# marcemq/crowdmod-ddpm-4D

Hardware: AMD Instinct MI355X
Metric: denoise-steps/sec (UNet fwd + sampler update) at ATC [B,4,T,H,W] (higher is better)
Workload: dtype f32; 1 GPU; config/ATC.yml sampling on the 12x36 grid, fp32 arithmetic (fp32 matrix instructions; fp32 products built from f16 two-way splits -- three v_mfma_f32_32x32x16_f16 cross terms, fp32 accumulate, same error against the reference as round 3's six-term bf16 form -- in the Winograd / quarter-resolution / last-conv layers, whose input is GroupNorm + SiLU output, and in the upsample layers, whose raw inpu; channels=4, past_len=5, future_len=3, global_batch=64, parallelism=batch-shard x1 (2 stream lanes of 32 chains per rank)

## Files before the change

crowdmod-ddpm-4d_amd/csrc/cm_conv_fin.hip:

```cpp
#include "cm_kernels.h"

#include <algorithm>
#include <cstring>
#include <vector>

namespace cm {

typedef float f32x16 __attribute__((ext_vector_type(16)));
typedef float f32x4 __attribute__((ext_vector_type(4)));
typedef __bf16 bf16x8 __attribute__((ext_vector_type(8)));
typedef _Float16 f16x8 __attribute__((ext_vector_type(8)));
typedef _Float16 f16x4 __attribute__((ext_vector_type(4)));

__device__ __forceinline__ float silu_f2(float v) { return v * __builtin_amdgcn_rcpf(1.0f + __expf(-v)); }

constexpr int FIN_ROWS = 64;
constexpr int FIN_PCOLS = 132;

template <int MODE>
__global__ __launch_bounds__(256, 2) void conv_fin_kernel(const ConvArgs a, const float *__restrict__ wfin, int ntx) {
  constexpr bool F16 = MODE == 1, H2 = MODE == 3;
  constexpr int U0 = MODE >= 2 ? 3 : 0, NTW = MODE >= 2 ? 2 : 3;
  constexpr int NTM = F16 ? 1 : 3;
  constexpr int RW = F16 ? 4 : 12;
  extern __shared__ __attribute__((aligned(16))) float lds[];
  float *A = lds;
  float *P = A + 4 * FIN_ROWS * RW;
  float *OACC = P + FIN_ROWS * FIN_PCOLS;
  const int tid = threadIdx.x, lane = tid & 63;
  const int wave = __builtin_amdgcn_readfirstlane(tid >> 6);
  const int r = lane & 31, hh = lane >> 5;
  const int BY = a.by, BX = a.bx, HX = BX + 2, HV = (BY + 2) * HX, NV = BY * BX;
  int tile = blockIdx.x;
  const int ntp = a.nty * ntx;
  const int b = tile / ntp, p = tile - b * ntp;
  const int ty = p / ntx, tx = p - ty * ntx;
  const int y0 = ty * BY, x0 = tx * BX;
  const size_t Vp = (size_t)a.Ys * a.Xs;
  const int C = a.C0;

  const int q = tid & 7;
  int soff[2];
  bool sok[2];
#pragma unroll
  for (int k = 0; k < 2; ++k) {
    const int hv = (tid >> 3) + 32 * k;
    const int hy = hv / HX, hx = hv - hy * HX;
    const int cy = y0 - 1 + hy, cx = x0 - 1 + hx;
    sok[k] = hv < HV && cy >= 0 && cy < a.Ys && cx >= 0 && cx < a.Xs;
    soff[k] = sok[k] ? cy * a.Xs + cx : 0;
  }
  f32x4 sc = {1.f, 1.f, 1.f, 1.f}, sh = {0.f, 0.f, 0.f, 0.f};
  if (a.gn) {
    const float *g = a.gn + (size_t)b * 2 * C + 4 * q;
    sc = *reinterpret_cast<const f32x4 *>(g);
    sh = *reinterpret_cast<const f32x4 *>(g + C);
  }
  const bool h16 = (a.h16 & 1) != 0;
  f32x4 ld[2];
  auto issue = [&](int z) {
    if (h16) {
      const _Float16 *sp = reinterpret_cast<const _Float16 *>(a.src0) + ((size_t)(b * a.Zs + z) * Vp) * C + 4 * q;
#pragma unroll
      for (int k = 0; k < 2; ++k) {
        const cm_f32x2_t two = *reinterpret_cast<const cm_f32x2_t *>(sp + (size_t)soff[k] * C);
        const f16x4 hv4 = __builtin_bit_cast(f16x4, two);
        ld[k] = f32x4{(float)hv4[0], (float)hv4[1], (float)hv4[2], (float)hv4[3]};
      }
    } else {
      const float *sp = a.src0 + ((size_t)(b * a.Zs + z) * Vp) * C + 4 * q;
#pragma unroll
      for (int k = 0; k < 2; ++k) ld[k] = *reinterpret_cast<const f32x4 *>(sp + (size_t)soff[k] * C);
    }
  };
  auto stage = [&]() {
#pragma unroll
    for (int k = 0; k < 2; ++k) {
      const int hv = (tid >> 3) + 32 * k;
      f32x4 w = ld[k];
      if (a.gn) {
        w = w * sc + sh;
        if (a.silu) { w[0] = silu_f2(w[0]); w[1] = silu_f2(w[1]); w[2] = silu_f2(w[2]); w[3] = silu_f2(w[3]); }
      }
      if (!sok[k]) w = f32x4{0.f, 0.f, 0.f, 0.f};
      float *dst = A + (size_t)(((q >> 1) & 1) * FIN_ROWS + hv) * RW + 2 * (q & 1) + (q >> 2) * (2 * FIN_ROWS * RW);
      if constexpr (F16) {
        const f16x4 hv4 = {(_Float16)w[0], (_Float16)w[1], (_Float16)w[2], (_Float16)w[3]};
        *reinterpret_cast<f16x4 *>(dst) = hv4;
      } else {
        cm_u32x2_t t3[3];
        if constexpr (H2) cm_split2_f16(w, t3);
        else cm_split3_bf16<NTW>(w, t3);
#pragma unroll
        for (int tm = 0; tm < NTW; ++tm) *reinterpret_cast<cm_u32x2_t *>(dst + 4 * tm) = t3[tm];
      }
    }
  };

  f32x4 bw[2][NTM];
#pragma unroll
  for (int ks = 0; ks < 2; ++ks)
#pragma unroll
    for (int tm = 0; tm < NTM; ++tm) bw[ks][tm] = reinterpret_cast<const f32x4 *>(wfin)[((size_t)(wave * 2 + ks) * NTM + tm) * 64 + lane];

  const int gu = tid & 63, dzg = tid >> 6;
  const bool gath = gu < NV && dzg < 3;
  const int guy = gu / BX, gux = gu - guy * BX;
  const int grow = guy * HX + gux;
  const int oy = y0 + guy, ox = x0 + gux;
  const bool oin = gath && oy < a.Yo && ox < a.Xo;
  f32x4 bias4 = {0.f, 0.f, 0.f, 0.f};
  if (gath && dzg >= 1) {
#pragma unroll
    for (int c = 0; c < 4; ++c) bias4[c] = c < a.Co ? a.bias[c] : 0.f;
  }
  for (int i = tid; i < 3 * 64 * 4; i += 256) OACC[i] = 0.f;

  const int Z = a.Zs;
  constexpr int TA[6] = {0, 2, 1, 0, 1, 0}, TB[6] = {2, 0, 1, 1, 0, 0};
  issue(0);
  stage();
  if (Z > 1) issue(1);
  __syncthreads();
  for (int z = 0; z < Z; ++z) {
    f32x16 acc[2];
#pragma unroll
    for (int j = 0; j < 2; ++j)
#pragma unroll
      for (int e = 0; e < 16; ++e) acc[j][e] = 0.f;
#pragma unroll
    for (int ks = 0; ks < 2; ++ks)
#pragma unroll
      for (int j = 0; j < 2; ++j) {
        const float *ap = A + (size_t)ks * (2 * FIN_ROWS * RW) + (size_t)(hh * FIN_ROWS + 32 * j + r) * RW;
        if constexpr (F16) {
          const f32x4 af = *reinterpret_cast<const f32x4 *>(ap);
          acc[j] = __builtin_amdgcn_mfma_f32_32x32x16_f16(__builtin_bit_cast(f16x8, bw[ks][0]), __builtin_bit_cast(f16x8, af), acc[j], 0, 0, 0);
        } else {
          f32x4 af[3];
#pragma unroll
          for (int tm = 0; tm < 3; ++tm) af[tm] = *reinterpret_cast<const f32x4 *>(ap + 4 * tm);
#pragma unroll
          for (int u = U0; u < 6; ++u) {
            if constexpr (H2)
              acc[j] = __builtin_amdgcn_mfma_f32_32x32x16_f16(__builtin_bit_cast(f16x8, bw[ks][TB[u]]), __builtin_bit_cast(f16x8, af[TA[u]]), acc[j], 0, 0, 0);
            else
              acc[j] = __builtin_amdgcn_mfma_f32_32x32x16_bf16(__builtin_bit_cast(bf16x8, bw[ks][TB[u]]), __builtin_bit_cast(bf16x8, af[TA[u]]), acc[j], 0, 0, 0);
          }
        }
      }
#pragma unroll
    for (int j = 0; j < 2; ++j)
#pragma unroll
      for (int g = 0; g < 4; ++g) {
        f32x4 pv = f32x4{acc[j][4 * g], acc[j][4 * g + 1], acc[j][4 * g + 2], acc[j][4 * g + 3]};
        if constexpr (H2) pv = pv * a.h2_oscale;
        *reinterpret_cast<f32x4 *>(P + (size_t)(32 * j + r) * FIN_PCOLS + 4 * (8 * wave + 2 * g + hh)) = pv;
      }
    __syncthreads();
    if (z + 1 < Z) {
      stage();
      if (z + 2 < Z) issue(z + 2);
    }
    if (gath) {
      const int zo = z + 1 - dzg;
      if (zo >= 0 && zo < a.Zo) {
        f32x4 s4 = {0.f, 0.f, 0.f, 0.f};
#pragma unroll
        for (int t9 = 0; t9 < 9; ++t9) {
          const int dy = t9 / 3, dx = t9 - 3 * dy;
          s4 += *reinterpret_cast<const f32x4 *>(P + (size_t)(grow + dy * HX + dx) * FIN_PCOLS + 4 * (dzg * 9 + t9));
        }
        float *oa = OACC + (size_t)(((zo % 3) * 64 + gu) * 4);
        f32x4 v = *reinterpret_cast<const f32x4 *>(oa) + s4;
        const bool last = dzg == 2 || (dzg == 1 && z == Z - 1);
        if (last) {
          if (oin) {
            float *o = a.out + ((size_t)((b * a.Zo + zo) * a.Yo + oy) * a.Xo + ox) * a.out_cs;
#pragma unroll
            for (int c = 0; c < 4; ++c)
              if (c < a.Co) o[c] = v[c] + bias4[c];
          }
          v = f32x4{0.f, 0.f, 0.f, 0.f};
        }
        *reinterpret_cast<f32x4 *>(oa) = v;
      }
    }
    __syncthreads();
  }
}

bool conv_fin_pick(int Y, int X, int *by, int *bx) {
  double best = 0;
  for (int y = 1; y <= Y; ++y)
    for (int x = 1; x <= X; ++x) {
      if (Y % y || X % x) continue;
      const int hv = (y + 2) * (x + 2);
      if (hv > FIN_ROWS || y * x > 64) continue;
      const double score = (double)(y * x) / FIN_ROWS;
      if (score > best) { best = score; *by = y; *bx = x; }
    }
  return best > 0;
}

bool conv_fin_ok(const ConvArgs &a) {
  return a.ntaps == 27 && a.td == 3 && a.stride == 1 && !a.par && !a.ups && a.C0 == 32 && a.C1 == 0 && a.Co >= 1 && a.Co <= 4 && !a.temb &&
         !a.resid && !a.stat_part && !a.pm && a.ks <= 1 && a.out_cs >= a.Co && a.Zs == a.Zo && a.Ys == a.Yo && a.Xs == a.Xo && a.by > 0 &&
         a.bx > 0 && a.Yo % a.by == 0 && a.Xo % a.bx == 0 && (a.by + 2) * (a.bx + 2) <= FIN_ROWS && a.by * a.bx <= 64 && !(a.h16 & ~1);
}

size_t conv_fin_lds(bool f16) {
  return ((size_t)2 * 2 * FIN_ROWS * (f16 ? 4 : 12) + (size_t)FIN_ROWS * FIN_PCOLS + 3 * 64 * 4) * sizeof(float);
}

hipError_t launch_conv_fin(const ConvArgs &a_in, const float *wfin, int mode, hipStream_t st) {
  ConvArgs a = a_in;
  a.dbg = conv_dbg_flags();
  if (!conv_fin_ok(a) || mode < 0 || mode > 3) return hipErrorInvalidValue;
  const int nty = a.Yo / a.by, ntx = a.Xo / a.bx;
  a.nty = nty;
  const dim3 grid((unsigned)(a.B * nty * ntx));
  const size_t lds = conv_fin_lds(mode == 1);
  static bool attr_set[64][4] = {{false}};
  int dev = 0;
  (void)hipGetDevice(&dev);
  const void *fn = mode == 1 ? reinterpret_cast<const void *>(conv_fin_kernel<1>)
                 : mode == 2 ? reinterpret_cast<const void *>(conv_fin_kernel<2>)
                 : mode == 3 ? reinterpret_cast<const void *>(conv_fin_kernel<3>) : reinterpret_cast<const void *>(conv_fin_kernel<0>);
  if (!attr_set[dev & 63][mode]) {
    hipError_t e = hipFuncSetAttribute(fn, hipFuncAttributeMaxDynamicSharedMemorySize, 160 * 1024);
    if (e != hipSuccess) return e;
    attr_set[dev & 63][mode] = true;
  }
  if (mode == 1) hipLaunchKernelGGL(conv_fin_kernel<1>, grid, dim3(256), lds, st, a, wfin, ntx);
  else if (mode == 2) hipLaunchKernelGGL(conv_fin_kernel<2>, grid, dim3(256), lds, st, a, wfin, ntx);
  else if (mode == 3) hipLaunchKernelGGL(conv_fin_kernel<3>, grid, dim3(256), lds, st, a, wfin, ntx);
  else hipLaunchKernelGGL(conv_fin_kernel<0>, grid, dim3(256), lds, st, a, wfin, ntx);
  return hipGetLastError();
}

__global__ __launch_bounds__(256) void fin_pack_kernel(const float *__restrict__ w, unsigned short *__restrict__ out, int Co, int f16, float wscale) {
  const int o = blockIdx.x * 256 + threadIdx.x;
  if (o >= 4 * 2 * 64 * 8) return;
  const int j = o & 7, lane = (o >> 3) & 63, ks = (o >> 9) & 1, nb = o >> 10;
  const int n = 32 * nb + (lane & 31), t = n >> 2, co = n & 3, ci = 16 * ks + 8 * (lane >> 5) + j;
  float v = 0.f;
  if (t < 27 && co < Co) {
    const int dz = t / 9, dy = (t / 3) % 3, dx = t % 3;
    v = w[((size_t)co * 32 + ci) * 27 + (dy * 3 + dx) * 3 + dz];
  }
  const int ntm = f16 == 1 ? 1 : 3;
  const size_t base = (((size_t)(nb * 2 + ks) * ntm) * 64 + lane) * 8 + j;
  if (f16 == 2) {
    const float vs = v * wscale;
    const _Float16 h = (_Float16)vs;
    const _Float16 md = (_Float16)(vs - (float)h);
    out[base] = __builtin_bit_cast(unsigned short, h);
    out[base + (size_t)64 * 8] = __builtin_bit_cast(unsigned short, md);
    out[base + (size_t)2 * 64 * 8] = 0;
  } else if (f16) {
    const _Float16 h = (_Float16)v;
    out[base] = __builtin_bit_cast(unsigned short, h);
  } else {
    float rem = v;
#pragma unroll
    for (int tm = 0; tm < 3; ++tm) {
      const __bf16 h = (__bf16)rem;
      out[base + (size_t)tm * 64 * 8] = __builtin_bit_cast(unsigned short, h);
      rem -= (float)h;
    }
  }
}

hipError_t launch_fin_pack(const float *w_ref, float *wfin, int Co, int mode, hipStream_t st, float wscale) {
  hipLaunchKernelGGL(fin_pack_kernel, dim3(16), dim3(256), 0, st, w_ref, reinterpret_cast<unsigned short *>(wfin), Co, mode, wscale);
  return hipGetLastError();
}

}
```

crowdmod-ddpm-4d_amd/csrc/cm_conv_io.hip:

```cpp
#include "cm_kernels.h"

namespace cm {

typedef float f32x16 __attribute__((ext_vector_type(16)));
typedef float f32x4 __attribute__((ext_vector_type(4)));
typedef float f32x2 __attribute__((ext_vector_type(2)));

template <int CIN>
__global__ __launch_bounds__(256) void conv_first_kernel(const ConvArgs a, const float *__restrict__ wpk, int nblk) {
  constexpr int NS = 27 * CIN / 2;
  constexpr int HC = CIN / 2;
  extern __shared__ __attribute__((aligned(16))) float lds[];
  const int tid = threadIdx.x, lane = tid & 63;
  const int wave = __builtin_amdgcn_readfirstlane(tid >> 6);
  const int r = lane & 31, hh = lane >> 5;
  int tile = blockIdx.x;
  if (!(gridDim.x & 7) && !(a.dbg & 4096)) tile = (tile & 7) * (int)(gridDim.x >> 3) + (tile >> 3);
  const int ty = tile % a.nty; tile /= a.nty;
  const int tz = tile % a.ntz;
  const int b = tile / a.ntz;
  const int nt = blockIdx.y;
  const int X = a.Xo, bz = a.bz, by = a.by;
  const int z0 = tz * bz, y0 = ty * by;
  const int HY = by + 2, HX = X + 2;
  const int HV = (bz + 2) * HY * HX;
  const int nbox = bz * by * X;

  int *outoff = reinterpret_cast<int *>(lds);
  float *P0 = lds + 32 * nblk;

  float wreg[NS];
  {
    const float *wp = wpk + (size_t)nt * NS * 64 + lane;
#pragma unroll
    for (int s = 0; s < NS; ++s) wreg[s] = wp[s * 64];
  }
  constexpr int SU = 4;
  for (int hv0 = tid; hv0 < HV; hv0 += 256 * SU) {
    f32x4 v0[SU], v1[CIN == 8 ? SU : 1];
    bool okv[SU];
#pragma unroll
    for (int u = 0; u < SU; ++u) {
      const int hv = min(hv0 + 256 * u, HV - 1);
      const int hz = hv / (HY * HX), rem = hv - hz * (HY * HX), hy = rem / HX, hx = rem - hy * HX;
      const int cz = z0 + hz - 1, cy = y0 + hy - 1, cx = hx - 1;
      const bool ok = cz >= 0 && cz < a.Zs && cy >= 0 && cy < a.Ys && cx >= 0 && cx < a.Xs;
      const float *sp = a.src0 + ((size_t)((b * a.Zs + (ok ? cz : 0)) * a.Ys + (ok ? cy : 0)) * a.Xs + (ok ? cx : 0)) * a.C0;
      v0[u] = *reinterpret_cast<const f32x4 *>(sp);
      if constexpr (CIN == 8) v1[u] = *reinterpret_cast<const f32x4 *>(sp + 4);
      okv[u] = ok;
    }
#pragma unroll
    for (int u = 0; u < SU; ++u) {
      const int hv = hv0 + 256 * u;
      if (hv >= HV) continue;
      const f32x4 z4 = {0.f, 0.f, 0.f, 0.f};
      const f32x4 w0 = okv[u] ? v0[u] : z4;
      if constexpr (CIN == 4) {
        *reinterpret_cast<f32x2 *>(P0 + hv * 2) = f32x2{w0[0], w0[1]};
        *reinterpret_cast<f32x2 *>(P0 + (HV + hv) * 2) = f32x2{w0[2], w0[3]};
      } else {
        const f32x4 w1 = okv[u] ? v1[u] : z4;
        *reinterpret_cast<f32x4 *>(P0 + hv * 4) = w0;
        *reinterpret_cast<f32x4 *>(P0 + (HV + hv) * 4) = w1;
      }
    }
  }
  for (int m = tid; m < 32 * nblk; m += 256) {
    int off = -1;
    if (m < nbox) {
      const int z = m / (by * X), rem = m - z * (by * X), y = rem / X, x = rem - y * X;
      const int oz = z0 + z, oy = y0 + y;
      if (oz < a.Zo && oy < a.Yo && b < a.B) off = ((b * a.Zo + oz) * a.Yo + oy) * a.Xo + x;
    }
    outoff[m] = off;
  }
  __syncthreads();

  const float *Ph = P0 + (size_t)hh * HV * HC;
  const int n = nt * 32 + r;
  const bool nok = n < a.Co;
  const float bias = a.bias[nok ? n : 0];
  for (int blk = wave; blk < nblk; blk += 4) {
    const int m = min(blk * 32 + r, nbox - 1);
    const int z = m / (by * X), rem = m - z * (by * X), y = rem / X, x = rem - y * X;
    const float *ap = Ph + (size_t)((z * HY + y) * HX + x) * HC;
    f32x16 acc;
#pragma unroll
    for (int i = 0; i < 16; ++i) acc[i] = 0.f;
#pragma unroll
    for (int t = 0; t < 27; ++t) {
      const int dz = t / 9, dy = (t / 3) % 3, dx = t % 3;
      const int toff = ((dz * HY + dy) * HX + dx) * HC;
      if constexpr (CIN == 4) {
        const f32x2 v = *reinterpret_cast<const f32x2 *>(ap + toff);
        acc = __builtin_amdgcn_mfma_f32_32x32x2f32(v[0], wreg[2 * t], acc, 0, 0, 0);
        acc = __builtin_amdgcn_mfma_f32_32x32x2f32(v[1], wreg[2 * t + 1], acc, 0, 0, 0);
      } else {
        const f32x4 v = *reinterpret_cast<const f32x4 *>(ap + toff);
#pragma unroll
        for (int jj = 0; jj < 4; ++jj) acc = __builtin_amdgcn_mfma_f32_32x32x2f32(v[jj], wreg[4 * t + jj], acc, 0, 0, 0);
      }
    }
    int offs[16];
    float rs[16];
#pragma unroll
    for (int reg = 0; reg < 16; ++reg) offs[reg] = outoff[blk * 32 + (reg & 3) + 8 * (reg >> 2) + 4 * hh];
#pragma unroll
    for (int reg = 0; reg < 16; ++reg) rs[reg] = acc[reg] + bias;
    if (a.h16 & 4) {
      _Float16 *oh = reinterpret_cast<_Float16 *>(a.out);
#pragma unroll
      for (int reg = 0; reg < 16; ++reg)
        if (nok && offs[reg] >= 0) oh[(size_t)offs[reg] * a.out_cs + n] = (_Float16)rs[reg];
    } else {
#pragma unroll
      for (int reg = 0; reg < 16; ++reg)
        if (nok && offs[reg] >= 0) a.out[(size_t)offs[reg] * a.out_cs + n] = rs[reg];
    }
    if (a.stat_part) {
      float s1 = 0.f, cnt = 0.f;
#pragma unroll
      for (int reg = 0; reg < 16; ++reg)
        if (offs[reg] >= 0) { s1 += rs[reg]; cnt += 1.f; }
      s1 += __shfl_xor(s1, 32);
      cnt += __shfl_xor(cnt, 32);
      const float mean = cnt > 0.f ? s1 / cnt : 0.f;
      float q = 0.f;
#pragma unroll
      for (int reg = 0; reg < 16; ++reg)
        if (offs[reg] >= 0) { const float d = rs[reg] - mean; q += d * d; }
      q += __shfl_xor(q, 32);
      const int slot = (tz * a.nty + ty) * nblk + blk;
      if (hh == 0 && nok && b < a.B) {
        float *sp = a.stat_part + (((size_t)b * a.stat_ns + slot) * a.stat_C + n) * 2;
        sp[0] = mean;
        sp[1] = q;
      }
      if (lane == 0 && n == 0 && b < a.B) a.stat_cnt[(size_t)b * a.stat_ns + slot] = cnt;
    }
  }
}

int conv_first_blocks(const ConvArgs &a) { return (a.bz * a.by * a.Xo + 31) / 32; }

size_t conv_first_lds(const ConvArgs &a, int cin) {
  const size_t HV = (size_t)(a.bz + 2) * (a.by + 2) * (a.Xo + 2);
  return ((size_t)32 * conv_first_blocks(a) + HV * cin) * sizeof(float);
}

bool conv_first_ok(const ConvArgs &a, int cin) {
  return a.ntaps == 27 && a.td == 3 && a.stride == 1 && !a.par && !a.ups && !a.gn && !a.temb && !a.resid && !a.src1 &&
         a.ks <= 1 && (cin == 4 || cin == 8) && a.C0 >= cin && a.C0 % 4 == 0 && a.bx == a.Xo && a.Xs == a.Xo &&
         conv_first_lds(a, cin) <= 64 * 1024;
}

hipError_t launch_conv_first(const ConvArgs &a_in, int cin, const float *wpk, hipStream_t st) {
  ConvArgs a = a_in;
  a.dbg = conv_dbg_flags();
  if (!conv_first_ok(a, cin)) return hipErrorInvalidValue;
  const int nblk = conv_first_blocks(a);
  const dim3 grid((unsigned)(a.B * a.ntz * a.nty), (unsigned)((a.Co + 31) / 32));
  const size_t lds = conv_first_lds(a, cin);
  if (cin == 4) hipLaunchKernelGGL(conv_first_kernel<4>, grid, dim3(256), lds, st, a, wpk, nblk);
  else hipLaunchKernelGGL(conv_first_kernel<8>, grid, dim3(256), lds, st, a, wpk, nblk);
  return hipGetLastError();
}

}
```

crowdmod-ddpm-4d_amd/csrc/cm_dit_host.inc:

```

struct cm_dit_plan {
  cm_dit_config cfg{};
  int Ns = 0, Tp = 0, qs = 0, tok = 0, Kp = 0, Nout = 0, ldmod = 0;
  float *X = nullptr, *QKV = nullptr, *AO = nullptr, *Hm = nullptr;
  float *modtab = nullptr;
  std::vector<const float *> w;
};

namespace {

constexpr int DIT_HEAD = 11;
constexpr int DIT_PER_BLOCK = 14;

void dit_build_params(cm_model *m) {
  const cm_dit_config &c = m->dit->cfg;
  const int64_t D = c.hidden_size, tx = D * c.time_multiple, p = c.patch_size, pt = c.t_patch_size;
  add_param(m, "spatial_pos_embed", {1, m->dit->Ns, D});
  add_param(m, "temporal_pos_embed", {1, c.t_max / pt, D});
  add_param(m, "dif_time_embeddings.time_blocks.0.weight", {TIME_ROWS, D});
  add_param(m, "dif_time_embeddings.time_blocks.1.weight", {tx, D});
  add_param(m, "dif_time_embeddings.time_blocks.1.bias", {tx});
  add_param(m, "dif_time_embeddings.time_blocks.3.weight", {tx, tx});
  add_param(m, "dif_time_embeddings.time_blocks.3.bias", {tx});
  add_param(m, "time_proj.0.weight", {D, tx});
// ... 89 lines not shown
  if (dev_alloc(m, (void **)&m->stage_past, B * per_past * sizeof(float))) return 1;
  CM_HIP(hipDeviceSynchronize());
  m->finalized = true;
  return 0;
}

int dit_forward(cm_model *m, int B, hipStream_t st, int b0) {
  const cm_dit_plan &d = *m->dit;
  const cm_dit_config &c = d.cfg;
  const int D = c.hidden_size, D3 = 3 * D, mlp = c.mlp_hidden, nq = d.Tp - d.qs;
  const long long r0 = (long long)b0 * d.tok, M = (long long)B * d.tok;
  const size_t vox = (size_t)m->L() * c.rows * c.cols * 8;
  float *X = d.X + r0 * D, *QKV = d.QKV + r0 * D3, *AO = d.AO + r0 * D, *Hm = d.Hm + r0 * mlp;
  cm::DitGemmArgs base{};
  base.tok = d.tok; base.tbuf = m->tbuf + b0; base.mod = d.modtab; base.ldmod = d.ldmod;
  base.L = m->L(); base.Hh = c.rows; base.Ww = c.cols; base.p = c.patch_size; base.pt = c.t_patch_size;
  base.Ns = d.Ns; base.wpn = c.cols / c.patch_size; base.Cout = c.out_channels;
  auto gemm = [&](int pro, int epi, long long rows, int N, int K) {
    cm::DitGemmArgs a = base;
    a.pro = pro; a.epi = epi; a.M = rows; a.N = N; a.K = K;
    a.grp = (int)rows;
    return a;
  };
  auto future_rows = [&](cm::DitGemmArgs &a, int slots) {
    a.M = (long long)B * slots * d.Ns; a.grp = slots * d.Ns; a.grp_stride = d.tok; a.grp_off = d.qs * d.Ns;
  };
  cm::DitGemmArgs a = gemm(cm::DIT_PRO_PATCH, cm::DIT_EPI_PATCH, M, D, d.Kp);
  a.x8 = m->x8 + (size_t)b0 * vox; a.W = d.w[9]; a.bias = d.w[10]; a.Y = X; a.ldy = D; a.spos = d.w[0]; a.tpos = d.w[1];
  CM_HIP(cm::launch_dit_gemm(a, st));
  cm::DitAttnArgs at{QKV, AO, B, d.Tp, d.Ns, d.qs, D, c.num_heads};
  for (int i = 0; i < c.depth; ++i) {
    const float *const *w = d.w.data() + DIT_HEAD + DIT_PER_BLOCK * i;
    const int mo = i * 9 * D;
    a = gemm(cm::DIT_PRO_LN, cm::DIT_EPI_BIAS, M, D3, D);
    a.A = X; a.lda = D; a.W = w[0]; a.bias = w[1]; a.Y = QKV; a.ldy = D3; a.off_shift = mo; a.off_scale = mo + D;
    CM_HIP(cm::launch_dit_gemm(a, st));
    CM_HIP(cm::launch_dit_attn_spatial(at, st));
    a = gemm(cm::DIT_PRO_NONE, cm::DIT_EPI_GATE, M, D, D);
    a.A = AO; a.lda = D; a.W = w[2]; a.bias = w[3]; a.Y = X; a.ldy = D; a.off_gate = mo + 2 * D;
    CM_HIP(cm::launch_dit_gemm(a, st));
    a = gemm(cm::DIT_PRO_LN, cm::DIT_EPI_BIAS, M, D3, D);
    a.A = X; a.lda = D; a.W = w[4]; a.bias = w[5]; a.Y = QKV; a.ldy = D3; a.off_shift = mo + 3 * D; a.off_scale = mo + 4 * D;
    CM_HIP(cm::launch_dit_gemm(a, st));
    CM_HIP(cm::launch_dit_attn_temporal(at, st));
    a = gemm(cm::DIT_PRO_NONE, cm::DIT_EPI_GATE, M, D, D);
    future_rows(a, nq);
    a.a_compact = 1; a.A = AO; a.lda = D; a.W = w[6]; a.bias = w[7]; a.Y = X; a.ldy = D; a.off_gate = mo + 5 * D;
    CM_HIP(cm::launch_dit_gemm(a, st));
    a = gemm(cm::DIT_PRO_LN, cm::DIT_EPI_GELU, M, mlp, D);
    a.A = X; a.lda = D; a.W = w[8]; a.bias = w[9]; a.Y = Hm; a.ldy = mlp; a.off_shift = mo + 6 * D; a.off_scale = mo + 7 * D;
    CM_HIP(cm::launch_dit_gemm(a, st));
    a = gemm(cm::DIT_PRO_NONE, cm::DIT_EPI_GATE, M, D, mlp);
    a.A = Hm; a.lda = mlp; a.W = w[10]; a.bias = w[11]; a.Y = X; a.ldy = D; a.off_gate = mo + 8 * D;
    CM_HIP(cm::launch_dit_gemm(a, st));
  }
  const float *const *wf = d.w.data() + DIT_HEAD + DIT_PER_BLOCK * c.depth;
  a = gemm(cm::DIT_PRO_LN, cm::DIT_EPI_UNPATCH, M, d.Nout, D);
  future_rows(a, nq);
  a.A = X; a.lda = D; a.W = wf[0]; a.bias = wf[1]; a.Y = m->eps_cl + (size_t)b0 * vox;
  a.off_shift = c.depth * 9 * D; a.off_scale = c.depth * 9 * D + D;
  CM_HIP(cm::launch_dit_gemm(a, st));
  return 0;
}

int dit_cost(const cm_model *m, int B, double *flops, double *bytes) {
  const cm_dit_plan &d = *m->dit;
  const cm_dit_config &c = d.cfg;
  const double D = c.hidden_size, mlp = c.mlp_hidden, tok = d.tok, Ns = d.Ns, Tp = d.Tp, nq = d.Tp - d.qs;
  double f = 2.0 * tok * d.Kp * D;
  const double blk = 2.0 * (2.0 * tok * D * 3.0 * D)
                     + 4.0 * Tp * Ns * Ns * D
                     + 2.0 * tok * D * D
                     + 4.0 * Ns * nq * Tp * D
                     + 2.0 * nq * Ns * D * D
                     + 2.0 * (2.0 * tok * D * mlp);
  f += c.depth * blk + 2.0 * nq * Ns * D * d.Nout;
  double wb = 0;
  for (const Param &p : m->params) wb += 4.0 * p.numel();
  if (flops) *flops = f * B;
  if (bytes) *bytes = wb + 4.0 * B * 2.0 * (double)m->L() * c.rows * c.cols * 8;
  return 0;
}

int denoise(cm_model *m, int B, hipStream_t st, int b0, int slab) {
  return m->dit ? dit_forward(m, B, st, b0) : run_ops(m, B, st, b0, slab);
}

}

extern "C" int cm_model_create_dit(const cm_dit_config *cfg, cm_model **out) {
  if (!cfg || !out) return fail("null argument");
  const cm_dit_config &c = *cfg;
  if (c.in_channels < 1 || c.in_channels > 8 || c.out_channels < 1 || c.out_channels > 8) return fail("in/out channels must be in [1,8]");
  if (c.max_batch < 1) return fail("max_batch must be >= 1");
  if (c.depth < 1 || c.time_multiple < 1 || c.past_len < 1 || c.future_len < 1) return fail("depth, time_multiple, past_len and future_len must be >= 1");
  if (c.patch_size < 1 || c.t_patch_size < 1) return fail("patch_size and t_patch_size must be >= 1");
  if (c.rows < 1 || c.cols < 1 || c.rows % c.patch_size || c.cols % c.patch_size)
    return fail("grid %dx%d is not divisible by patch_size %d (DiT4D_V4.py:25-28)", c.rows, c.cols, c.patch_size);
  const int L = c.past_len + c.future_len;
  if (L % c.t_patch_size) return fail("past_len + future_len = %d is not divisible by t_patch_size %d (DiT4D_V4.py:257)", L, c.t_patch_size);
  const int Tp = L / c.t_patch_size, tslots = c.t_max / c.t_patch_size;
  if (Tp > tslots) return fail("T_p = %d temporal slots exceed the %d rows of temporal_pos_embed (t_max %d / t_patch_size %d)", Tp, tslots, c.t_max, c.t_patch_size);
  if (c.num_heads < 1 || c.hidden_size < 1 || c.hidden_size % c.num_heads)
    return fail("hidden_size %d is not divisible by num_heads %d", c.hidden_size, c.num_heads);
  if (c.hidden_size / c.num_heads != 64) return fail("head dim %d: the DiT attention kernels are built for head dim 64", c.hidden_size / c.num_heads);
  if (c.mlp_hidden < 64 || c.mlp_hidden % 64) return fail("mlp_hidden %d must be a positive multiple of 64", c.mlp_hidden);
  const int Ns = (c.rows / c.patch_size) * (c.cols / c.patch_size);
  if (Ns > 64) return fail("%d spatial patches: the spatial attention kernel holds at most 64", Ns);
  if (Tp > 8) return fail("%d temporal slots: the temporal attention kernel holds at most 8", Tp);
  if (c.past_len / c.t_patch_size >= Tp) return fail("no future temporal slot: past_len / t_patch_size = %d of %d", c.past_len / c.t_patch_size, Tp);
  if (c.device >= 0) {
    int ndev = 0;
    CM_HIP(hipGetDeviceCount(&ndev));
    if (c.device >= ndev) return fail("device %d not available (%d devices)", c.device, ndev);
  }
  auto m = std::make_unique<cm_model>();
  m->cfg.in_channels = c.in_channels; m->cfg.out_channels = c.out_channels;
  m->cfg.rows = c.rows; m->cfg.cols = c.cols; m->cfg.past_len = c.past_len; m->cfg.future_len = c.future_len;
  m->cfg.time_multiple = c.time_multiple; m->cfg.max_batch = c.max_batch; m->cfg.device = c.device;
  m->device = c.device;
  m->dit = new cm_dit_plan;
  cm_dit_plan &d = *m->dit;
  d.cfg = c;
  d.Ns = Ns; d.Tp = Tp; d.qs = c.past_len / c.t_patch_size; d.tok = Tp * Ns;
  d.Kp = c.in_channels * c.t_patch_size * c.patch_size * c.patch_size;
  d.Nout = c.t_patch_size * c.out_channels * c.patch_size * c.patch_size;
  d.ldmod = c.depth * 9 * c.hidden_size + 2 * c.hidden_size;
  dit_build_params(m.get());
  if (m->device >= 0) {
    DevGuard g(m->device);
    CM_HIP(hipStreamCreateWithFlags(&m->stream, hipStreamNonBlocking));
    for (int i = 1; i < 4; ++i) {
      CM_HIP(hipStreamCreateWithFlags(&m->lane_stream[i], hipStreamNonBlocking));
      CM_HIP(hipEventCreateWithFlags(&m->ev_join[i], hipEventDisableTiming));
    }
    CM_HIP(hipEventCreateWithFlags(&m->ev_fork, hipEventDisableTiming));
  }
  *out = m.release();
  return 0;
}
```

crowdmod-ddpm-4d_amd/csrc/cm_host_selftest.cpp:

```cpp
#include "cm_model.cpp"

#include <cstdlib>
#include <random>

namespace {

int g_checks = 0;
#define EXPECT(cond)                                                                  \
  do {                                                                                \
    ++g_checks;                                                                       \
    if (!(cond)) { fprintf(stderr, "selftest FAILED: %s (%s:%d)\n", #cond, __FILE__, __LINE__); exit(1); } \
  } while (0)

void test_schedule() {
  for (int T : {2, 3, 50, 1000}) {
    cm_schedule *s = nullptr;
    EXPECT(cm_schedule_create(T, 0.5f, 1e-4f, 2e-2f, -1, &s) == 0);
    std::vector<float> buf((size_t)T);
    for (int w = 0; w < 6; ++w) EXPECT(cm_schedule_table(s, w, buf.data(), T) == 0);
    EXPECT(cm_schedule_table(s, 6, buf.data(), T) != 0);
    EXPECT(cm_schedule_table(s, 0, buf.data(), T - 1) != 0);
    cm_sample_opts o{};
    int32_t n = 0;
    o.sampler = CM_SAMPLER_DDPM;
// ... 355 lines not shown
      grid(2, 3, 9, 128, 384); a.ntaps = 1; a.td = 1; a.CK = 128; op.cls = K_CONV1; op.NB = 2;
      if (rc == RC_1X1_STATS) op.stat_act = &out;
      else if (p16) op.d_w1x1_16 = frag;
      op.skip_if_fused = rc == RC_SKIP_ABSORBED;
      break;
  }
  return op;
}

void test_conv_route() {
  struct Want { ConvKernel kernel; ConvForm form; };
  const ConvKernel QR = CONV_QR, KS = CONV_KSPLIT, UPS = CONV_UPS, F16D = CONV_F16D, WINO = CONV_WINO, FIRST = CONV_FIRST, FIN = CONV_FIN,
                   X11 = CONV_1X1_F16, GEN = CONV_GENERIC, NONE = CONV_NONE;
  const ConvForm FP32 = FORM_FP32, F16 = FORM_F16, B6 = FORM_B6, B3 = FORM_B3, H2 = FORM_H2;
  const Want want[RC_COUNT][6] = {
       {{WINO, H2}, {WINO, B6}, {WINO, B3}, {F16D, F16}, {WINO, B6}, {WINO, FP32}},
       {{WINO, H2}, {WINO, B6}, {WINO, B3}, {F16D, F16}, {WINO, B6}, {WINO, FP32}},
       {{WINO, H2}, {WINO, B6}, {WINO, B3}, {F16D, F16}, {WINO, B6}, {WINO, FP32}},
       {{WINO, H2}, {WINO, B6}, {WINO, B3}, {F16D, F16}, {WINO, B6}, {WINO, FP32}},
       {{QR, H2}, {QR, B6}, {QR, B3}, {QR, FP32}, {QR, B6}, {KS, FP32}},
       {{QR, H2}, {QR, B6}, {QR, B3}, {QR, FP32}, {KS, FP32}, {KS, FP32}},
       {{KS, FP32}, {KS, FP32}, {KS, FP32}, {KS, FP32}, {KS, FP32}, {KS, FP32}},
       {{GEN, FP32}, {GEN, FP32}, {GEN, FP32}, {GEN, FP32}, {GEN, FP32}, {GEN, FP32}},
       {{UPS, H2}, {UPS, B6}, {UPS, B3}, {UPS, F16}, {UPS, B6}, {UPS, FP32}},
       {{UPS, B6}, {UPS, B6}, {UPS, B3}, {UPS, F16}, {UPS, B6}, {UPS, FP32}},
       {{FIRST, FP32}, {FIRST, FP32}, {FIRST, FP32}, {FIRST, FP32}, {FIRST, FP32}, {FIRST, FP32}},
       {{FIN, H2}, {FIN, B6}, {FIN, B3}, {FIN, F16}, {FIN, B6}, {FIN, B6}},
       {{GEN, FP32}, {GEN, FP32}, {GEN, FP32}, {X11, F16}, {GEN, FP32}, {GEN, FP32}},
       {{GEN, FP32}, {GEN, FP32}, {GEN, FP32}, {GEN, FP32}, {GEN, FP32}, {GEN, FP32}},
       {{NONE, FP32}, {NONE, FP32}, {NONE, FP32}, {NONE, FP32}, {GEN, FP32}, {GEN, FP32}},
  };
  const int plans[4] = {CM_PRECISION_F32, CM_PRECISION_F32X, CM_PRECISION_F32R, CM_PRECISION_F16};
  int walked = 0;
  for (int rc = 0; rc < RC_COUNT; ++rc)
    for (int pi = 0; pi < 4; ++pi)
      for (int train = 0; train < 2; ++train)
        for (int stale = 0; stale < 2; ++stale)
          for (int off = 0; off < 2; ++off)
            for (int dbg = 0; dbg < 3; ++dbg) {
              Op op = route_class_op(rc, plans[pi]);
              op.h2_off = off; op.dbg_raw = dbg >= 1; op.dbg_h2 = dbg == 2;
              const bool src_stats = rc != RC_UPS_NO_STATS;
              const ConvRoute r = conv_route(op, plans[pi], train, stale, src_stats);
              ++walked;
              const bool h2_live = !stale && !off && dbg != 1;
              const Want w = train ? want[rc][pi == 3 ? 5 : 4] : want[rc][(pi == 0 && !h2_live) ? 1 : pi];
              EXPECT(r.kernel == w.kernel && r.form == w.form);
              if (r.form == FORM_H2) EXPECT(plans[pi] == CM_PRECISION_F32 && !train && !stale && !off && (!op.dbg_raw || op.dbg_h2) &&
                                            (op.d_wwino_h2 || op.d_wqr_h2 || op.d_wfin_h2 || (op.d_wups_h2 && src_stats)));
              if (train) EXPECT(r.form != FORM_F16 && r.form != FORM_B3 && r.kernel != CONV_F16D && r.kernel != CONV_1X1_F16 && r.kernel != CONV_NONE);
              if (train && r.kernel == CONV_QR) EXPECT(op.train_qr && op.d_wqr_b6);
              if (op.ks > 1) EXPECT(r.kernel == CONV_QR || r.kernel == CONV_KSPLIT);
              EXPECT(r.kernel == conv_route(op, plans[pi], train, false).kernel);
              for (int mask = 1; mask < 64; ++mask) {
                const bool takes = r.kernel == CONV_F16D || (r.kernel == CONV_UPS && r.form == FORM_F16 && !(mask & ~(1 | 4))) ||
                                   (r.kernel == CONV_FIRST && mask == 4) || ((r.kernel == CONV_FIN || r.kernel == CONV_SMALLN) && !(mask & ~(1 | 2)));
                EXPECT(route_takes_h16(r, mask) == takes);
              }
            }
  {
    Op op = route_class_op(RC_LAST, CM_PRECISION_F32);
    op.pm_off = 0;
    EXPECT(conv_route(op, CM_PRECISION_F32, true, false).kernel == CONV_SMALLN && conv_route(op, CM_PRECISION_F32, false, false).kernel == CONV_FIN);
    op.ca.C1 = 32;
    EXPECT(conv_route(op, CM_PRECISION_F32, false, false).kernel == CONV_SMALLN);
    walked += 3;
  }
  {
    Op op = route_class_op(RC_UPS_STATS, CM_PRECISION_F16);
    op.d_wups16 = nullptr;
    op.MB = 5; op.NB = 1; op.ca.bz = 4; op.ca.by = 6; op.ca.bx = 6;
    ConvRoute r = conv_route(op, CM_PRECISION_F16, false, false);
    EXPECT(r.kernel == CONV_GENERIC && r.form == FORM_F16);
    op.ca.bx = 5;
    r = conv_route(op, CM_PRECISION_F16, false, false);
    EXPECT(r.kernel == CONV_GENERIC && r.form == FORM_FP32);
    r = conv_route(op, CM_PRECISION_F16, true, false);
    EXPECT(r.kernel == CONV_UPS && r.form == FORM_FP32);
    walked += 3;
  }
  printf("test_conv_route: %d combinations walked\n", walked);
}

void test_misc_errors() {
  EXPECT(cm_abi_version() == CM_ABI_VERSION);
  EXPECT(cm_device_count(nullptr) != 0);
  EXPECT(cm_model_destroy(nullptr) == 0);
  EXPECT(cm_schedule_destroy(nullptr) == 0);
  EXPECT(cm_train_set_lr(nullptr, 1.f) != 0);
  EXPECT(cm_train_set_sample_base(nullptr, 0) != 0);
  int32_t n = 0;
  EXPECT(cm_model_num_params(nullptr, &n) != 0);
  EXPECT(cm_profile_enable(nullptr, 1) != 0);
  EXPECT(cm_frame_metrics(0, nullptr, nullptr, 1, 1, 1, 1, 1, nullptr, nullptr) != 0);
  EXPECT(std::string(cm_last_error()).size() > 0);
  EXPECT(linspace_f32(0.f, 1.f, 10, 0) == 0.f && linspace_f32(0.f, 1.f, 10, 9) == 1.f && linspace_f32(3.f, 5.f, 1, 0) == 3.f);
}

}

int main() {
  test_schedule();
  test_plan_and_params();
  test_packers();
  test_tile_planner();
  test_round3_packers();
  test_wino_form_dispatch();
  test_conv_route();
  test_misc_errors();
  printf("selftest ok: %d checks\n", g_checks);
  return 0;
}
```

crowdmod-ddpm-4d_amd/csrc/cm_kernels.h:

```cpp
#pragma once
#include <hip/hip_runtime.h>
#include <stdint.h>
#include <stdlib.h>
#include <vector>

namespace cm {

inline const char *diag_env(const char *name) {
  static const bool on = [] { const char *d = getenv("CM_DIAG"); return d && d[0] == '1' && d[1] == 0; }();
  return on ? getenv(name) : nullptr;
}

#ifdef __HIPCC__
typedef float cm_f32x2_t __attribute__((ext_vector_type(2)));
typedef float cm_f32x4_t __attribute__((ext_vector_type(4)));
typedef __bf16 cm_bf16x2_t __attribute__((ext_vector_type(2)));
typedef unsigned cm_u32x2_t __attribute__((ext_vector_type(2)));
typedef _Float16 cm_f16x4_t __attribute__((ext_vector_type(4)));
__device__ __forceinline__ unsigned cm_cvt_pk_bf16(float a, float b) {
  const cm_f32x2_t v = {a, b};
  return __builtin_bit_cast(unsigned, __builtin_convertvector(v, cm_bf16x2_t));
}
template <int NT = 3>
__device__ __forceinline__ void cm_split3_bf16(cm_f32x4_t x, cm_u32x2_t (&t)[3]) {
#pragma unroll
  for (int tm = 0; tm < NT; ++tm) {
    const unsigned p01 = cm_cvt_pk_bf16(x[0], x[1]), p23 = cm_cvt_pk_bf16(x[2], x[3]);
    t[tm] = cm_u32x2_t{p01, p23};
    if (tm < NT - 1) {
      x[0] -= __uint_as_float(p01 << 16); x[1] -= __uint_as_float(p01 & 0xffff0000u);
      x[2] -= __uint_as_float(p23 << 16); x[3] -= __uint_as_float(p23 & 0xffff0000u);
    }
  }
}
typedef _Float16 cm_f16x2_t __attribute__((ext_vector_type(2)));
__device__ __forceinline__ void cm_split2_f16(cm_f32x4_t x, cm_u32x2_t (&t)[3]) {
  const cm_f32x2_t a = {x[0], x[1]}, b = {x[2], x[3]};
  const cm_f16x2_t ha = __builtin_convertvector(a, cm_f16x2_t), hb = __builtin_convertvector(b, cm_f16x2_t);
  t[0] = cm_u32x2_t{__builtin_bit_cast(unsigned, ha), __builtin_bit_cast(unsigned, hb)};
  const cm_f32x2_t ra = a - __builtin_convertvector(ha, cm_f32x2_t), rb = b - __builtin_convertvector(hb, cm_f32x2_t);
  const cm_f16x2_t ma = __builtin_convertvector(ra, cm_f16x2_t), mb = __builtin_convertvector(rb, cm_f16x2_t);
  t[1] = cm_u32x2_t{__builtin_bit_cast(unsigned, ma), __builtin_bit_cast(unsigned, mb)};
}
#endif

struct ConvArgs {
  const float *src0;
  const float *src1;
  int C0, C1;
  const float *gn;
  int silu;
  const float *pm;
  int pm_stride;
  const float *wfrag;
  const float *bias;
  const float *temb;
  int temb_stride;
  const long long *tidx;
  const float *resid;
  int res_cs;
  float *out;
  int out_cs;
  int Co;
  int B;
  int Zs, Ys, Xs;
  int Zo, Yo, Xo;
  int ntaps;
  int td;
  int par;
  long long wpar_stride;
  int ks;
  long long kpart;
  int stride;
  int ups;
  int bs, bz, by, bx;
  int nts, ntz, nty, ntx;
  int CK;
  int nch0, nch1;
  const int *hvtab;
  const int *mtab;
  float *stat_part;
  float *stat_cnt;
  int stat_C, stat_ns;
  const float *s2src0; const float *s2src1;
  int s2C0, s2C1;
  const float *s2w;
  int dbg;
  float *dbg_buf;
  int stagger;
  int f16;
  int zsplit;
  int h16;
  float h2_oscale;
  alignas(8) unsigned char layout_pad[40];
  const float *gs_gamma, *gs_beta;
  int gs_groups;
  float gs_eps;
  const float *gp0, *gc0, *gp1, *gc1;
  int gns0, gns1;
};
#ifdef __HIPCC__
__device__ __forceinline__ void cm_chan_combine(float &n, float &mean, float &m2, float nb, float meanb, float m2b) {
  if (nb == 0.f) return;
  const float nt = n + nb;
  const float d = meanb - mean;
  const float f = nb * __builtin_amdgcn_rcpf(nt);
  mean += d * f;
  m2 += m2b + d * d * n * f;
  n = nt;
}
__device__ __forceinline__ void cm_gn_rows_from_slots(const ConvArgs &a, int b, int V, float *rows, float *scratch, int tid, int nth) {
  const int Ctot = a.C0 + a.C1, cg = Ctot / a.gs_groups;
  for (int c = tid; c < Ctot; c += nth) {
    const bool s0 = c < a.C0;
    const float *p = s0 ? a.gp0 : a.gp1, *nn = s0 ? a.gc0 : a.gc1;
    const int ns = s0 ? a.gns0 : a.gns1, Cx = s0 ? a.C0 : a.C1, cc = s0 ? c : c - a.C0;
    float N = 0.f, M = 0.f, S2 = 0.f;
    for (int s8 = 0; s8 < ns; s8 += 8) {
      float cn[8];
      cm_f32x2_t q[8];
#pragma unroll
      for (int u = 0; u < 8; ++u) {
        const int sl = s8 + u < ns ? s8 + u : ns - 1;
        cn[u] = s8 + u < ns ? nn[(size_t)b * ns + sl] : 0.f;
        q[u] = *reinterpret_cast<const cm_f32x2_t *>(p + (((size_t)b * ns + sl) * Cx + cc) * 2);
      }
#pragma unroll
      for (int u = 0; u < 8; ++u) cm_chan_combine(N, M, S2, cn[u], q[u][0], q[u][1]);
    }
    scratch[2 * c] = M;
    scratch[2 * c + 1] = S2;
  }
  __syncthreads();
  for (int c = tid; c < Ctot; c += nth) {
    const int g0 = (c / cg) * cg;
    float N = 0.f, M = 0.f, S2 = 0.f;
    for (int k = g0; k < g0 + cg; ++k) cm_chan_combine(N, M, S2, (float)V, scratch[2 * k], scratch[2 * k + 1]);
    const float rstd = rsqrtf(S2 / N + a.gs_eps);
    const float sc = rstd * a.gs_gamma[c];
    rows[c] = sc;
    rows[Ctot + c] = a.gs_beta[c] - M * sc;
  }
}
__device__ __forceinline__ float cm_h2_sample_scale(const float *__restrict__ gp, const float *__restrict__ gc, int ns, int C, int b,
                                                    float *scratch, int tid, int nth) {
  float bm = 0.f;
  for (int c = tid; c < C; c += nth) {
    float N = 0.f, M = 0.f, S2 = 0.f;
    for (int s8 = 0; s8 < ns; s8 += 8) {
      float cn[8];
      cm_f32x2_t q[8];
#pragma unroll
      for (int u = 0; u < 8; ++u) {
        const int sl = s8 + u < ns ? s8 + u : ns - 1;
        cn[u] = s8 + u < ns ? gc[(size_t)b * ns + sl] : 0.f;
        q[u] = *reinterpret_cast<const cm_f32x2_t *>(gp + (((size_t)b * ns + sl) * C + c) * 2);
      }
#pragma unroll
      for (int u = 0; u < 8; ++u) cm_chan_combine(N, M, S2, cn[u], q[u][0], q[u][1]);
    }
    bm = fmaxf(bm, fabsf(M) + sqrtf(fmaxf(S2, 0.f)));
  }
#pragma unroll
  for (int off = 32; off >= 1; off >>= 1) bm = fmaxf(bm, __shfl_xor(bm, off));
  if ((tid & 63) == 0) scratch[tid >> 6] = bm;
  __syncthreads();
  float m = scratch[0];
  for (int w = 1; w < (nth >> 6); ++w) m = fmaxf(m, scratch[w]);
  __syncthreads();
  const unsigned e = (__float_as_uint(m) >> 23) & 255u;
  int se = 267 - (int)e;
  se = se < 32 ? 32 : (se > 222 ? 222 : se);
  if (!(m > 0.f) || e == 255u) se = 127;
  return __uint_as_float((unsigned)se << 23);
}
#endif

// ... 6 lines not shown
void conv_build_tables(const ConvArgs &a, int MB, int *hvtab , int *mtab );
int conv_halo_voxels(const ConvArgs &a);
hipError_t launch_conv(const ConvArgs &a, int MB, int NB, hipStream_t st);
bool conv1x1_f16_ok(const ConvArgs &a, int NB);
hipError_t launch_conv1x1_f16(const ConvArgs &a, int NB, hipStream_t st);
bool conv_variant_exists(int MB, int NB);
bool conv_ups_pick(int Z, int Y, int X, int *tz, int *ty, int *tx, int *mbw, int *planes);
bool conv_ups_ok(const ConvArgs &a, int mbw, int planes, int nbp);
int conv_ups_slots(const ConvArgs &a, int mbw);
hipError_t launch_conv_ups(const ConvArgs &a, int mbw, int planes, int nbp, hipStream_t st);
hipError_t launch_ups_b6_repack(const float *wfrag, long long wpar_stride, float *w6, long long w6_stride, int Co, int Ci, int NBP, hipStream_t st);
bool conv_smalln_ok(const ConvArgs &a, int MB);
size_t conv_smalln_lds(const ConvArgs &a, int MB);
hipError_t launch_conv_smalln(const ConvArgs &a, int MB, const float *wsm, hipStream_t st);

bool conv_first_ok(const ConvArgs &a, int cin);
int conv_first_blocks(const ConvArgs &a);
size_t conv_first_lds(const ConvArgs &a, int cin);
hipError_t launch_conv_first(const ConvArgs &a, int cin, const float *wpk, hipStream_t st);

bool conv_wino_tile_ok(int bz, int by, int bx);
bool conv_wino_ok(const ConvArgs &a);
size_t conv_wino_lds(int bz, int by, int bx, bool f16, int nbw);
int conv_wino_nbw(int bz, int Co);
int conv_wino_nbw_run(const ConvArgs &a, bool f16);
bool conv_wino_two_step(int bz, int by, int bx, bool f16, int nbw);
bool conv_wino_p_taken(const ConvArgs &a, bool f16, bool own_gn);
enum { WINO_FORM_ONE = 1, WINO_FORM_PLAIN = 2, WINO_FORM_OWNGN = 4, WINO_FORM_WHOLE = 8 };
int conv_wino_form(const ConvArgs &a, int G);
void conv_wino_form_counts(long long counts[16], bool reset);
hipError_t launch_conv_wino(const ConvArgs &a, bool f16, hipStream_t st);
bool conv_wino_b6_ok(int bz, int by, int bx, int Co, int Zo);
hipError_t launch_wino_b6_repack(const float *wwino, float *w6, long long n_floats, hipStream_t st);
hipError_t launch_wgrad_wino(const ConvArgs &a, const float *dy, int dy_cs, float *part, int G, int ncb, int nkb, hipStream_t st);
hipError_t launch_wgrad_wino_reduce(const float *part, int G, int ncb, int nkb, int Co, int Ci, float *dW, hipStream_t st);
bool conv_wino_pick(int Zo, int Yo, int Xo, int *bz, int *by, int *bx);

struct QrArgs {
  const float *src0, *src1;
  int C0, C1;
  const float *part0, *cnt0;
  int ns0;
  const float *part1, *cnt1;
  int ns1;
  const float *gamma, *beta;
  int groups;
  float eps;
  int silu;
  float *gn_out;
  const float *wq6;
  int three;
  float h2_oscale;
  const float *wq;
  const float *bias;
  const float *temb;
  int temb_stride;
  const long long *tidx;
  const float *resid;
  int res_cs;
  float *out;
  int out_cs, Co, B, Y, X;
  float *stat_part, *stat_cnt;
  int stat_C;
  const float *s2src0, *s2src1;
  int s2C0, s2C1;
  const float *s2w;
  int qshift;
  const float *pm;
  int pm_stride;
  int raw;
};
bool conv_qr_ok(const QrArgs &a);
bool conv_qr2_b6_ok(const QrArgs &a);
hipError_t launch_qr_b6_repack(const float *wq, float *wq6, long long n_floats, int Ci, hipStream_t st);
hipError_t launch_conv_qr(const QrArgs &a, hipStream_t st);

bool conv_f16d_pick(int Z, int Y, int X, int *bz, int *by, int *bx, int *mbw);
bool conv_f16d_ok(const ConvArgs &a, int mbw);
int conv_f16d_slots(const ConvArgs &a, int mbw);
hipError_t launch_conv_f16d(const ConvArgs &a, int mbw, hipStream_t st);

bool conv_fin_pick(int Y, int X, int *by, int *bx);
bool conv_fin_ok(const ConvArgs &a);
hipError_t launch_conv_fin(const ConvArgs &a, const float *wfin, int mode , hipStream_t st);
hipError_t launch_fin_pack(const float *w_ref , float *wfin, int Co, int mode , hipStream_t st, float wscale = 1.f);
constexpr size_t CM_FIN_W_FLOATS = 4 * 2 * 3 * 64 * 4;

hipError_t launch_chan_stats(const float *x, int B, int V, int C, int nslice, float *part, float *cnt, hipStream_t st);
hipError_t launch_gn_finalize(const float *part0, const float *cnt0, int ns0, int C0, const float *part1,
                              const float *cnt1, int ns1, int C1, int V, const float *gamma, const float *beta,
                              int groups, float eps, float *gn, float *mr, int B, hipStream_t st);
struct CombineArgs {
  const float *part; int S; long long stride;
  const float *bias; const float *temb; int temb_stride; const long long *tidx;
  const float *resid; int res_cs;
  float *out; int C, V, B;
  float *stat_part; float *stat_cnt; int nslots;
  const float *fin_gamma, *fin_beta; float *fin_gn, *fin_mr;
  const float *fin_p1, *fin_n1; int fin_ns1, fin_C1, fin_groups; float fin_eps;
};
hipError_t launch_ksplit_combine(const CombineArgs &a, hipStream_t st);
bool combine_gn_ok(const CombineArgs &a);
hipError_t launch_combine_gn(const CombineArgs &a, hipStream_t st);
hipError_t launch_assemble_input(const float *past, const float *future, float *x8, int B, int C, int H, int W,
                                 int P, int F, int which , hipStream_t st);
hipError_t launch_extract_output(const float *eps_cl, int cs, float *out, int B, int C, int H, int W, int P, int F,
                                 hipStream_t st);
hipError_t launch_time_mlp(const float *table, const float *W1, const float *b1, const float *W2, const float *b2,
                           const float *Wd, const float *bd, int te, int tx, int nproj, int nrows, float *temb_raw,
                           float *out, const long long *rowidx, hipStream_t st);
hipError_t launch_attn_core(const float *qkv, float *out, int B, int S, int E, int heads, hipStream_t st);
hipError_t launch_attn_core_f16(const float *qkv, float *out, int B, int S, int E, int heads, hipStream_t st);

struct AttnBlockArgs {
  const float *x;
  const float *gamma, *beta;
  const float *w_in, *b_in;
  const float *w_out;
  float *part;
  int B, S, E, heads, groups;
  float eps;
};
bool attn_block_ok(int S, int E, int heads, int groups);
size_t attn_block_lds_bytes(int S, int E, int heads);
hipError_t launch_attn_block(const AttnBlockArgs &a, hipStream_t st);

enum { DIT_PRO_NONE = 0, DIT_PRO_LN = 1, DIT_PRO_PATCH = 2 };
enum { DIT_EPI_BIAS = 0, DIT_EPI_SILU = 1, DIT_EPI_SILU2 = 2, DIT_EPI_GELU = 3, DIT_EPI_GATE = 4, DIT_EPI_PATCH = 5,
       DIT_EPI_UNPATCH = 6 };
struct DitGemmArgs {
  int pro, epi;
  const float *A; int lda;
  const float *W, *bias;
  float *Y; int ldy;
  long long M; int N, K;
  int grp, grp_stride, grp_off;
  int a_compact;
  int tok;
  const long long *tbuf;
  const float *mod; int ldmod;
  int off_shift, off_scale, off_gate;
  const float *x8;
  const float *spos, *tpos;
  int L, Hh, Ww, p, pt, Ns, wpn, Cout;
};
struct DitAttnArgs {
  const float *qkv;
  float *out;
  int B, Tp, Ns, qs, E, heads;
};
hipError_t launch_dit_gemm(const DitGemmArgs &a, hipStream_t st);
hipError_t launch_dit_attn_spatial(const DitAttnArgs &a, hipStream_t st);
hipError_t launch_dit_attn_temporal(const DitAttnArgs &a, hipStream_t st);

struct StepRow { int t; float c_x, c_eps, c_noise, guid; int draw; int step; float mass; };
struct StepArgs {
  float *x;
  const float *eps_cl;
  int cs;
  float *x8;
  const float *noise;
  float *hist;
  int B, C, H, W, P, F;
  float c_x, c_eps, c_noise;
  float guid;
  unsigned long long seed;
  long long sample_id_base;
  int step;
  int draw;
  const StepRow *tab; const int *kctr;
  long long row_stride;
  long long boff;
  long long *t_next; long long t_next_v;
};
hipError_t launch_sampler_step(const StepArgs &a, hipStream_t st);
hipError_t launch_mass_grad(const float *x, int Cin, float *q, int Cout, int B, int H, int W, int L, float delta_t,
                            float delta_l, float eps, hipStream_t st);
struct MassApplyArgs {
  float *x;
  const float *q;
  float *x8;
  float *hist;
  int B, C, H, W, P, F;
  float c;
  const StepRow *tab; const int *kctr;
  long long row_stride, boff;
};
hipError_t launch_mass_apply(const MassApplyArgs &a, hipStream_t st);
hipError_t launch_q_sample(const float *x0, const long long *t, const float *eps, const float *sab, const float *s1m,
                           float *xt, int B, long long per, hipStream_t st);
hipError_t launch_fill_t(long long *t, int B, long long value, hipStream_t st);
hipError_t launch_count_nonfinite(const float *x, long long n, int *count, hipStream_t st);
hipError_t launch_step_begin(long long *t, int B, const StepRow *tab, int *kctr, hipStream_t st);
struct WgradPackArgs {
  const float *wide; int wide_cs;
  const float *gn; int silu;
  const float *narrow; int narrow_cs;
  int cn_valid, mirror;
  int B, Z, Y, X;
  int bz, by, bx, ntz, nty, ntx;
  float *part;
};
hipError_t launch_wgrad_pack(const WgradPackArgs &a, int CN, int G, hipStream_t st);
hipError_t launch_wgrad_pack_reduce(const float *part, int G, int CN, int cn_valid, int mirror, int Co, int Ci, float *dW, hipStream_t st);

hipError_t launch_wgrad_1x1(const ConvArgs &a, const float *dy, int dy_cs, long long V, float *part, int G, int ncb, int nkb, int NKB, hipStream_t st);

hipError_t launch_wgrad_par(const ConvArgs &a, const float *dy, int dy_cs, float *part, int G, int ncb, int nkb, hipStream_t st);

bool wgrad_zs_ok(const ConvArgs &a);
hipError_t launch_wgrad_zs(const ConvArgs &a, const float *dy, int dy_cs, float *part, int G, int ncb, int nkb, hipStream_t st);

struct VsumJob { const float *x; int V, C, cs; float *out; int ostride; float *out2; int ostride2; };
hipError_t launch_voxel_sum_jobs(const VsumJob *jobs, int njobs, int B, int maxC, hipStream_t st);

struct CopyJob { float *dst; const float *src; long long n; };
hipError_t launch_copy_jobs(const CopyJob *jobs, int njobs, long long max_n, hipStream_t st);

struct BsumJob { const float *in; float *out; int C, stride; };
hipError_t launch_batch_sum_jobs(const BsumJob *jobs, int njobs, int B, int maxC, hipStream_t st);
hipError_t launch_mse_loss(const float *a, const float *b, long long n, float *partial, float *loss, hipStream_t st);
hipError_t launch_dropout_mask(float *mask, int B, int C, float p, unsigned long long seed, long long sample_id_base,
                               int step, hipStream_t st);
hipError_t launch_randn(float *x, int B, long long per, unsigned long long seed, long long sample_id_base, int step,
                        hipStream_t st);
hipError_t launch_frame_metrics(const float *pred, const float *gt, int N, int C, int H, int W, int F, double *out,
                                float *minmax, hipStream_t st);
hipError_t launch_cl_to_ref(const float *x_cl, int cs, float *out, int B, int C, int Z, int Y, int X, hipStream_t st);

hipError_t launch_wgrad(const ConvArgs &a, int MB, const float *dy, int dy_cs, float *part, int G, int ncb, int nkb,
                        hipStream_t st);
hipError_t launch_wgrad_reduce(const float *part, int G, int ncb, int nkb, int ntaps, int Co, int Ci, float *dW,
                               hipStream_t st, int force_nvs = 0 );
hipError_t launch_wgrad_reduce_par(const float *part, int G, int ncb, int nkb, int Co, int Ci, float *dW, hipStream_t st);
hipError_t launch_voxel_sum(const float *x, int B, int V, int C, int cs, float *out, int ostride,
                            float *scratch , hipStream_t st);
hipError_t launch_batch_sum(const float *in, int B, int C, int stride, float *out, int accumulate, hipStream_t st);
struct GnbArgs {
  const float *x0; const float *x1; int C0, C1;
  const float *dA; int dA_cs;
  const float *gn;
  const float *mr;
  const float *gamma;
  const float *pm; int pm_stride;
  int silu;
  int V, B, groups;
  float *part;
  int nsl;
  float *coef;
  float *dgb;
  float *g0; float *g1; int acc0, acc1;
};
hipError_t launch_gn_backward(const GnbArgs &a, hipStream_t st);
hipError_t launch_add_into(float *dst, int dcs, const float *src, int scs, int C, long long rows, int accumulate,
                           hipStream_t st);
hipError_t launch_upsample2(const float *x, float *y, int B, int Z, int Y, int X, int C, hipStream_t st);
hipError_t launch_sumpool2(const float *y, float *x, int B, int Z, int Y, int X, int C, int accumulate, hipStream_t st);
hipError_t launch_zero_stuff2(const float *y, float *u, int B, int Z, int Y, int X, int C, hipStream_t st);
// ... 24 lines not shown
```

crowdmod-ddpm-4d_amd/csrc/cm_misc.hip:

```cpp
#include "cm_kernels.h"

namespace cm {

typedef float f32x4 __attribute__((ext_vector_type(4)));

__device__ __forceinline__ float silu_f(float v) { return v / (1.0f + __expf(-v)); }

__device__ __forceinline__ void chan_combine(float &n, float &mean, float &m2, float nb, float meanb, float m2b) {
  if (nb == 0.f) return;
  const float nt = n + nb;
  const float d = meanb - mean;
  const float f = nb * __builtin_amdgcn_rcpf(nt);
  mean += d * f;
  m2 += m2b + d * d * n * f;
  n = nt;
}

__global__ __launch_bounds__(256) void chan_stats_kernel(const float *__restrict__ x, int V, int C, int nslice,
                                                         float *__restrict__ part, float *__restrict__ cnt) {
  __shared__ float sh[256 * 4 * 3];
  const int b = blockIdx.y, sl = blockIdx.x;
  const int Q = C >> 2;
  const int tid = threadIdx.x;
  const int vs = (V + nslice - 1) / nslice;
// ... 657 lines not shown
  const float scale = rsqrtf((float)D);
  for (int qb = wave; qb < nkb; qb += 4) {
    const int q = qb * 32 + r, qc = q < S ? q : S - 1;
    f16x8m qf[2];
#pragma unroll
    for (int g = 0; g < 2; ++g) {
      const float *qp = base + (size_t)qc * 3 * E + hd * D + 16 * g + 8 * hh;
      const f32x4 q0 = *reinterpret_cast<const f32x4 *>(qp) * scale, q1 = *reinterpret_cast<const f32x4 *>(qp + 4) * scale;
      qf[g] = f16x8m{(_Float16)q0[0], (_Float16)q0[1], (_Float16)q0[2], (_Float16)q0[3],
                     (_Float16)q1[0], (_Float16)q1[1], (_Float16)q1[2], (_Float16)q1[3]};
    }
    f32x16m o;
#pragma unroll
    for (int i = 0; i < 16; ++i) o[i] = 0.f;
    float mx = -3.0e38f, l = 0.f;
    for (int kb = 0; kb < nkb; ++kb) {
      f32x16m sc;
#pragma unroll
      for (int i = 0; i < 16; ++i) sc[i] = 0.f;
#pragma unroll
      for (int g = 0; g < 2; ++g) {
        const f16x8m kf = *reinterpret_cast<const f16x8m *>(Ks + (size_t)(kb * 32 + r) * KS + 16 * g + 8 * hh);
        sc = __builtin_amdgcn_mfma_f32_32x32x16_f16(kf, qf[g], sc, 0, 0, 0);
      }
      float bm = -3.0e38f;
#pragma unroll
      for (int reg = 0; reg < 16; ++reg) {
        const int key = kb * 32 + (reg & 3) + 8 * (reg >> 2) + 4 * hh;
        if (key >= S) sc[reg] = -3.0e38f;
        bm = fmaxf(bm, sc[reg]);
      }
      bm = fmaxf(bm, __shfl_xor(bm, 32));
      const float mnew = fmaxf(mx, bm);
      const float corr = __expf(mx - mnew);
      mx = mnew;
      l *= corr;
#pragma unroll
      for (int i = 0; i < 16; ++i) o[i] *= corr;
      float ps = 0.f;
      f16x8m pf[2];
#pragma unroll
      for (int reg = 0; reg < 16; ++reg) {
        const int key = kb * 32 + (reg & 3) + 8 * (reg >> 2) + 4 * hh;
        const float pv = key < S ? __expf(sc[reg] - mnew) : 0.f;
        ps += pv;
        pf[reg >> 3][reg & 7] = (_Float16)pv;
      }
      l += ps;
#pragma unroll
      for (int u = 0; u < 2; ++u) {
        const _Float16 *vp = Vt + (size_t)r * VS + kb * 32 + 16 * u + 4 * hh;
        const f16x4m v0 = *reinterpret_cast<const f16x4m *>(vp), v1 = *reinterpret_cast<const f16x4m *>(vp + 8);
        const f16x8m vf = {v0[0], v0[1], v0[2], v0[3], v1[0], v1[1], v1[2], v1[3]};
        o = __builtin_amdgcn_mfma_f32_32x32x16_f16(vf, pf[u], o, 0, 0, 0);
      }
    }
    l += __shfl_xor(l, 32);
    if (q < S) {
      const float inv = 1.0f / l;
      float *op = out + ((size_t)b * S + q) * E + hd * D;
#pragma unroll
      for (int reg = 0; reg < 16; ++reg) op[(reg & 3) + 8 * (reg >> 2) + 4 * hh] = o[reg] * inv;
    }
  }
}

hipError_t launch_attn_core_f16(const float *qkv, float *out, int B, int S, int E, int heads, hipStream_t st) {
  if (heads <= 0 || E / heads != 32 || E % heads || S < 1) return hipErrorInvalidValue;
  const int Sp = (S + 31) / 32 * 32;
  const size_t smem = ((size_t)Sp * (32 + 8) + (size_t)32 * (Sp + 8)) * sizeof(_Float16);
  if (smem > 160 * 1024) return hipErrorInvalidValue;
  static bool attr_set[64] = {false};
  int dev = 0;
  (void)hipGetDevice(&dev);
  if (!attr_set[dev & 63]) {
    hipError_t e = hipFuncSetAttribute(reinterpret_cast<const void *>(attn_core_f16_kernel), hipFuncAttributeMaxDynamicSharedMemorySize, 160 * 1024);
    if (e != hipSuccess) return e;
    attr_set[dev & 63] = true;
  }
  hipLaunchKernelGGL(attn_core_f16_kernel, dim3(heads, B), dim3(256), smem, st, qkv, out, S, E);
  return hipGetLastError();
}

__device__ __forceinline__ void philox4x32_10(unsigned c0, unsigned c1, unsigned c2, unsigned c3, unsigned k0,
                                              unsigned k1, unsigned out[4]) {
#pragma unroll
  for (int i = 0; i < 10; ++i) {
    const unsigned long long p0 = 0xD2511F53ull * c0;
    const unsigned long long p1 = 0xCD9E8D57ull * c2;
    const unsigned n0 = (unsigned)(p1 >> 32) ^ c1 ^ k0;
    const unsigned n1 = (unsigned)p1;
    const unsigned n2 = (unsigned)(p0 >> 32) ^ c3 ^ k1;
    const unsigned n3 = (unsigned)p0;
    c0 = n0; c1 = n1; c2 = n2; c3 = n3;
    k0 += 0x9E3779B9u;
    k1 += 0xBB67AE85u;
  }
  out[0] = c0; out[1] = c1; out[2] = c2; out[3] = c3;
}

__device__ __forceinline__ float philox_normal(unsigned long long seed, long long sample, int step, long long elem) {
  unsigned r[4];
  philox4x32_10((unsigned)(elem >> 1), (unsigned)sample, (unsigned)step, (unsigned)((sample >> 32) ^ 0x5eed),
                (unsigned)seed, (unsigned)(seed >> 32), r);
  const float u1 = ((float)(r[0] >> 8) + 0.5f) * (1.0f / 16777216.0f);
  const float u2 = ((float)(r[1] >> 8) + 0.5f) * (1.0f / 16777216.0f);
  const float rad = sqrtf(-2.0f * __logf(u1));
  const float ang = 6.283185307179586f * u2;
  return (elem & 1) ? rad * __sinf(ang) : rad * __cosf(ang);
}

__global__ __launch_bounds__(256) void randn_kernel(float *__restrict__ x, long long per, long long total,
                                                    unsigned long long seed, long long sample_id_base, int step) {
  const long long i = (long long)blockIdx.x * 256 + threadIdx.x;
  if (i >= total) return;
  const long long b = i / per, e = i - b * per;
  x[i] = philox_normal(seed, sample_id_base + b, step, e);
}

hipError_t launch_randn(float *x, int B, long long per, unsigned long long seed, long long sample_id_base, int step,
                        hipStream_t st) {
  const long long total = (long long)B * per;
  hipLaunchKernelGGL(randn_kernel, dim3((unsigned)((total + 255) / 256)), dim3(256), 0, st, x, per, total, seed,
                     sample_id_base, step);
  return hipGetLastError();
}

__global__ __launch_bounds__(256) void sampler_step_kernel(StepArgs a) {
  if (a.tab) {
    const int k = *a.kctr;
    const StepRow r = a.tab[k];
    a.c_x = r.c_x; a.c_eps = r.c_eps; a.c_noise = r.c_noise; a.guid = r.guid; a.draw = r.draw; a.step = r.step;
    if (a.noise) a.noise += (long long)k * a.row_stride + a.boff;
    if (a.hist) a.hist += (long long)(k + 1) * a.row_stride + a.boff;
  }
  const long long per = (long long)a.C * a.H * a.W * a.F;
  const long long total = per * a.B;
  const long long i = (long long)blockIdx.x * 256 + threadIdx.x;
  if (a.t_next && i < a.B) a.t_next[i] = a.t_next_v;
  if (i >= total) return;
  const long long b = i / per, e = i - b * per;
  const int f = (int)(e % a.F);
  long long q = e / a.F;
  const int w = (int)(q % a.W); q /= a.W;
  const int hh = (int)(q % a.H);
  const int c = (int)(q / a.H);
  const int L = a.P + a.F;
  const size_t cl = ((((size_t)b * L + (a.P + f)) * a.H + hh) * a.W + w);
  const float eps = a.eps_cl[cl * a.cs + c];
  float z = 0.f;
  if (a.draw) z = a.noise ? a.noise[i] : philox_normal(a.seed, a.sample_id_base + b, a.step, e);
  float xn = a.c_x * a.x[i] + a.c_eps * eps + a.c_noise * z;
  if (a.guid != 0.f && c == 0) xn -= a.guid * (xn > 0.f ? 1.f : (xn < 0.f ? -1.f : 0.f));
  a.x[i] = xn;
  if (a.x8) a.x8[cl * 8 + c] = xn;
  if (a.hist) a.hist[i] = xn;
}

hipError_t launch_sampler_step(const StepArgs &a, hipStream_t st) {
  const long long total = (long long)a.B * a.C * a.H * a.W * a.F;
  hipLaunchKernelGGL(sampler_step_kernel, dim3((unsigned)((total + 255) / 256)), dim3(256), 0, st, a);
  return hipGetLastError();
}

__global__ __launch_bounds__(256) void q_sample_kernel(const float *__restrict__ x0, const long long *__restrict__ t,
                                                       const float *__restrict__ eps, const float *__restrict__ sab,
                                                       const float *__restrict__ s1m, float *__restrict__ xt,
                                                       long long per, long long total) {
  const long long i = (long long)blockIdx.x * 256 + threadIdx.x;
  if (i >= total) return;
  const long long b = i / per;
  const long long tt = t[b];
  xt[i] = sab[tt] * x0[i] + s1m[tt] * eps[i];
}

hipError_t launch_q_sample(const float *x0, const long long *t, const float *eps, const float *sab, const float *s1m,
                           float *xt, int B, long long per, hipStream_t st) {
  const long long total = (long long)B * per;
  hipLaunchKernelGGL(q_sample_kernel, dim3((unsigned)((total + 255) / 256)), dim3(256), 0, st, x0, t, eps, sab, s1m,
                     xt, per, total);
  return hipGetLastError();
}

__global__ __launch_bounds__(256) void mse_partial_kernel(const float *__restrict__ a, const float *__restrict__ b,
                                                          long long n, float *__restrict__ partial) {
  __shared__ float sh[256];
  float acc = 0.f;
  for (long long i = (long long)blockIdx.x * 256 + threadIdx.x; i < n; i += (long long)gridDim.x * 256) {
    const float d = a[i] - b[i];
    acc = fmaf(d, d, acc);
  }
  sh[threadIdx.x] = acc;
  __syncthreads();
  for (int s = 128; s > 0; s >>= 1) {
    if ((int)threadIdx.x < s) sh[threadIdx.x] += sh[threadIdx.x + s];
    __syncthreads();
  }
  if (threadIdx.x == 0) partial[blockIdx.x] = sh[0];
}

__global__ void mse_final_kernel(const float *__restrict__ partial, int np, long long n, float *__restrict__ loss) {
  if (threadIdx.x == 0 && blockIdx.x == 0) {
    double s = 0.0;
    for (int i = 0; i < np; ++i) s += (double)partial[i];
    *loss = (float)(s / (double)n);
  }
}

hipError_t launch_mse_loss(const float *a, const float *b, long long n, float *partial, float *loss, hipStream_t st) {
  const int np = 64;
  hipLaunchKernelGGL(mse_partial_kernel, dim3(np), dim3(256), 0, st, a, b, n, partial);
  hipLaunchKernelGGL(mse_final_kernel, dim3(1), dim3(64), 0, st, partial, np, n, loss);
  return hipGetLastError();
}

__global__ void dropout_mask_kernel(float *__restrict__ mask, int B, int C, float p, unsigned long long seed,
                                    long long sample_id_base, int step) {
  const int i = blockIdx.x * 256 + threadIdx.x;
  if (i >= B * C) return;
  const int b = i / C, c = i - b * C;
  unsigned r[4];
  philox4x32_10((unsigned)c, (unsigned)(sample_id_base + b), (unsigned)step, 0xD120u, (unsigned)seed,
                (unsigned)(seed >> 32), r);
  const float u = ((float)(r[0] >> 8) + 0.5f) * (1.0f / 16777216.0f);
  mask[i] = (u >= p) ? 1.0f / (1.0f - p) : 0.0f;
}

hipError_t launch_dropout_mask(float *mask, int B, int C, float p, unsigned long long seed, long long sample_id_base,
                               int step, hipStream_t st) {
  hipLaunchKernelGGL(dropout_mask_kernel, dim3((B * C + 255) / 256), dim3(256), 0, st, mask, B, C, p, seed,
                     sample_id_base, step);
  return hipGetLastError();
}

__global__ void fill_t_kernel(long long *t, int B, long long v) {
  const int i = blockIdx.x * 256 + threadIdx.x;
  if (i < B) t[i] = v;
}

// ... 38 lines not shown
```

crowdmod-ddpm-4d_amd/csrc/cm_model.cpp:

```cpp
#include <hip/hip_runtime.h>

#include <algorithm>
#include <cmath>
#include <cstdarg>
#include <cstdio>
#include <cstring>
#include <map>
#include <memory>
#include <string>
#include <thread>
#include <vector>

#include "../../include/crowdmod_hip.h"
#include "cm_kernels.h"

namespace {

thread_local std::string g_err;

int fail(const char *fmt, ...) {
  char buf[1024];
  va_list ap;
  va_start(ap, fmt);
  vsnprintf(buf, sizeof(buf), fmt, ap);
// ... 107 lines not shown
  float *d_wsmall = nullptr;
  int small_nco = 4;
  bool fin = false;
  int fin_by = 0, fin_bx = 0;
  float *d_wfin = nullptr, *d_wfin16 = nullptr, *d_wfin_src = nullptr;
  float *d_zero_bias = nullptr;
  const Act *out_act = nullptr, *resid_act = nullptr;
  double flops_per_sample = 0;
  std::string label;
  double prof_ms = 0;
  int64_t prof_n = 0;
  mutable int prof_B = 0;
  const Act *act = nullptr;
  const Act *g0 = nullptr, *g1 = nullptr;
  const float *gamma = nullptr, *beta = nullptr;
  float *gn_out = nullptr;
  float *gn_mr = nullptr;
  std::string gname, bename;
  const float *qkv = nullptr;
  float *aout = nullptr;
  int S = 0, E = 0;
  bool in_attn_block = false;
  const Act *ab_x = nullptr;
  Act *ab_out = nullptr;
  int ab_gn = -1, ab_qkv = -1, ab_outc = -1;
  float *d_win = nullptr, *d_wout = nullptr;
  std::string win_name, wout_name;
};

}

struct cm_schedule {
  int T = 0;
  int device = 0;
  std::vector<float> tab[6];
  float *d_sab = nullptr, *d_s1m = nullptr;
};

struct cm_train_state;
struct cm_dit_plan;
void cm_free_train_state(cm_train_state *t);
struct cm_model {
  cm_unet_config cfg{};
  cm_dit_plan *dit = nullptr;
  int device = 0;
  hipStream_t stream = nullptr;
  hipStream_t lane_stream[4] = {nullptr, nullptr, nullptr, nullptr};
  hipEvent_t ev_join[4] = {nullptr, nullptr, nullptr, nullptr}, ev_fork = nullptr;
  std::vector<Param> params;
  std::map<std::string, int> pindex;
  std::vector<BlockDesc> enc, bott, dec;
  int final_ch = 0;
  bool finalized = false;
  int precision = CM_PRECISION_F32;

  std::vector<void *> allocs;
  std::vector<std::unique_ptr<Act>> acts;
  std::map<std::string, Act *> act_by_name;
  std::vector<Op> ops;
  std::map<std::string, float *> dparam;

  float *x8 = nullptr;
  Act *x8_act = nullptr;
  float *eps_cl = nullptr;
  long long *tbuf = nullptr;
  float *temb_table = nullptr;
  int nproj = 0;
  float *d_time[7] = {nullptr};
  struct cm_train_state *train = nullptr;
  float *dropmask = nullptr;
  bool train_fwd = false;
  bool h2_stale = false;
  float *train_temb = nullptr;
  long long *train_iota = nullptr;
  bool use_train_temb = false;
  float *mse_partial = nullptr, *mse_loss = nullptr;
  float *ks_scratch = nullptr;
  size_t ks_scratch_floats = 0;
  float *xstate = nullptr;
  cm::StepRow *d_steptab = nullptr;
  size_t steptab_cap = 0;
  int *d_kctr = nullptr;
  int *d_nonfinite = nullptr;
  float *mass_q = nullptr;
  float *stage_past = nullptr, *stage_fut = nullptr, *stage_out = nullptr;
  float *stage_noise = nullptr;
  size_t stage_noise_cap = 0;
  float *stage_hist = nullptr;
  size_t stage_hist_cap = 0;

  bool profile = false;
  float prof_ms[K_NCLASS] = {0};
  int64_t prof_n[K_NCLASS] = {0};
  std::vector<std::pair<int, std::pair<hipEvent_t, hipEvent_t>>> prof_events[4];
  hipEvent_t prof_base = nullptr;
  float prof_union_ms[8] = {0, 0, 0, 0, 0, 0, 0, 0};

  int L() const { return cfg.past_len + cfg.future_len; }
  int64_t per_sample() const { return (int64_t)cfg.in_channels * cfg.rows * cfg.cols * cfg.future_len; }
};

namespace {
int refresh_h2(cm_model *m);

void add_param(cm_model *m, const std::string &name, std::vector<int64_t> shape) {
  Param p;
  p.name = name;
  p.shape = std::move(shape);
  p.host.assign((size_t)p.numel(), 0.f);
  m->pindex[name] = (int)m->params.size();
  m->params.push_back(std::move(p));
}

void build_plan(cm_model *m) {
  const cm_unet_config &c = m->cfg;
  const int base = c.base_channels, nres = c.n_levels;
  const int64_t te = base, tx = (int64_t)base * c.time_multiple;
  add_param(m, "time_embeddings.time_blocks.0.weight", {TIME_ROWS, te});
  add_param(m, "time_embeddings.time_blocks.1.weight", {tx, te});
  add_param(m, "time_embeddings.time_blocks.1.bias", {tx});
  add_param(m, "time_embeddings.time_blocks.3.weight", {tx, tx});
  add_param(m, "time_embeddings.time_blocks.3.bias", {tx});
  add_param(m, "first.weight", {base, c.in_channels, 3, 3, 3});
  add_param(m, "first.bias", {base});

  std::vector<int> stack{base};
  int cin = base, idx = 0;
  for (int level = 0; level < nres; ++level) {
    const int cout = base * c.channel_mult[level];
    for (int r = 0; r < c.num_res_blocks; ++r) {
      m->enc.push_back({0, "encoder_blocks." + std::to_string(idx++), cin, cout, c.apply_attention[level] != 0, 0, level});
      cin = cout;
      stack.push_back(cin);
    }
    if (level != nres - 1) {
      m->enc.push_back({1, "encoder_blocks." + std::to_string(idx++), cin, cin, 0, 0, level});
      stack.push_back(cin);
    }
  }
  m->bott.push_back({0, "bottleneck_blocks.0", cin, cin, 1, 0, nres - 1});
  m->bott.push_back({0, "bottleneck_blocks.1", cin, cin, 0, 0, nres - 1});
  idx = 0;
  for (int level = nres - 1; level >= 0; --level) {
    const int cout = base * c.channel_mult[level];
    for (int r = 0; r < c.num_res_blocks + 1; ++r) {
      const int skip = stack.back();
      stack.pop_back();
      m->dec.push_back({0, "decoder_blocks." + std::to_string(idx++), skip + cin, cout, c.apply_attention[level] != 0, skip, level});
      cin = cout;
    }
    if (level != 0) m->dec.push_back({2, "decoder_blocks." + std::to_string(idx++), cin, cin, 0, 0, level});
  }
  m->final_ch = cin;

  auto add_block_params = [&](const BlockDesc &b) {
    const std::string &p = b.prefix;
    if (b.kind == 0) {
      add_param(m, p + ".normalize_1.weight", {b.cin});
      add_param(m, p + ".normalize_1.bias", {b.cin});
      add_param(m, p + ".conv_1.weight", {b.cout, b.cin, 3, 3, 3});
      add_param(m, p + ".conv_1.bias", {b.cout});
      add_param(m, p + ".dense_1.weight", {b.cout, tx});
      add_param(m, p + ".dense_1.bias", {b.cout});
      add_param(m, p + ".normalize_2.weight", {b.cout});
      add_param(m, p + ".normalize_2.bias", {b.cout});
      add_param(m, p + ".conv_2.weight", {b.cout, b.cout, 3, 3, 3});
// ... 1034 lines not shown
    }
  }
  if (op.first_k) {
    const cm::ConvArgs keep = op.ca;
    pick_tile_first(op);
    if (cm::conv_first_ok(op.ca, op.first_cin)) return 0;
    op.ca = keep;
    op.first_k = false;
  }
  pick_tile(op, TUNE_BATCH);
  std::vector<int> hv((size_t)cm::conv_halo_voxels(op.ca)), mt((size_t)32 * op.MB);
  if (hv.size() > 16384) return fail("halo box too large");
  cm::conv_build_tables(op.ca, op.MB, hv.data(), mt.data());
  if (dev_alloc(m, (void **)&op.d_hvtab, 16384 * sizeof(int))) return 1;
  if (dev_alloc(m, (void **)&op.d_mtab, 256 * sizeof(int))) return 1;
  CM_HIP(hipMemcpyAsync(op.d_hvtab, hv.data(), hv.size() * sizeof(int), hipMemcpyHostToDevice, m->stream));
  CM_HIP(hipMemcpyAsync(op.d_mtab, mt.data(), mt.size() * sizeof(int), hipMemcpyHostToDevice, m->stream));
  CM_HIP(hipStreamSynchronize(m->stream));
  op.ca.hvtab = op.d_hvtab;
  op.ca.mtab = op.d_mtab;
  return 0;
}

enum ConvKernel { CONV_NONE, CONV_QR, CONV_KSPLIT, CONV_UPS, CONV_F16D, CONV_WINO, CONV_FIRST, CONV_FIN, CONV_SMALLN, CONV_1X1_F16, CONV_GENERIC };
const char *const kConvKernelName[] = {"none", "qr", "ksplit", "ups", "f16d", "wino", "first", "fin", "smalln", "1x1_f16", "generic"};
enum ConvForm { FORM_FP32 = 0, FORM_F16 = 1, FORM_B6 = 2, FORM_B3 = 3, FORM_H2 = 4 };
struct ConvRoute { ConvKernel kernel; ConvForm form; };

int h16_mask(const Op &op, bool train_fwd) {
  auto is16 = [&](const Act *t) { return t && t->h16 && !train_fwd; };
  const int io = (is16(op.in0) ? 1 : 0) | (is16(op.in1) ? 2 : 0) | (is16(op.out_act) ? 4 : 0);
  if (op.d_s2w && !train_fwd) return io | (is16(op.skip0) ? 16 : 0) | (is16(op.skip1) ? 32 : 0);
  return io | (is16(op.resid_act) ? 8 : 0);
}

ConvRoute conv_route(const Op &op, int precision, bool train_fwd, bool h2_stale, bool ups_src_stats = true) {
  static const bool no_train_qr = cm::diag_env("CM_NO_TRAIN_QR") != nullptr, no_train_b6 = cm::diag_env("CM_NO_TRAIN_B6") != nullptr;
  const bool infer = !train_fwd;
  const bool six_ok = infer || !no_train_b6;
  const ConvForm six = (precision == CM_PRECISION_F32R && infer) ? FORM_B3 : FORM_B6;
  const bool h2 = precision == CM_PRECISION_F32 && infer && !h2_stale && !op.h2_off && (!op.dbg_raw || op.dbg_h2);
  auto form = [&](const float *w16, const float *w6, const float *wh2) {
    return (w16 && infer) ? FORM_F16 : !w6 ? FORM_FP32 : (h2 && wh2) ? FORM_H2 : six;
  };
  const cm::ConvArgs &g = op.ca;
  if (op.skip_if_fused && infer) return {CONV_NONE, FORM_FP32};
  if (op.qr && (infer || (op.d_wqr_b6 && op.train_qr && !no_train_qr))) {
    cm::QrArgs q{};
    q.C0 = g.C0; q.C1 = g.C1; q.Co = g.Co; q.Y = g.Yo; q.X = g.Xo; q.groups = GN_GROUPS; q.raw = 1; q.wq6 = op.d_wqr_b6;
    return {CONV_QR, form(nullptr, cm::conv_qr2_b6_ok(q) ? op.d_wqr_b6 : nullptr, op.d_wqr_h2)};
  }
  if (op.ks > 1) return {CONV_KSPLIT, FORM_FP32};
  if (op.ups && (op.d_wups16 || !(op.d_wfrag16 && infer)))
    return {CONV_UPS, form(op.d_wups16, six_ok ? op.d_wups_b6 : nullptr, ups_src_stats ? op.d_wups_h2 : nullptr)};
  if (op.wino && op.f16d && infer) return {CONV_F16D, FORM_F16};
  if (op.wino)
    return {CONV_WINO, form(op.d_wwino16, (op.d_wwino_b6 && six_ok && cm::conv_wino_b6_ok(g.bz, g.by, g.bx, g.Co, g.Zo)) ? op.d_wwino_b6 : nullptr, op.d_wwino_h2)};
  if (op.first_k) return {CONV_FIRST, FORM_FP32};
  static float set;
  cm::ConvArgs a = g;
  a.stat_part = op.stat_act ? &set : nullptr;
  a.pm = (train_fwd && op.pm_off >= 0) ? &set : nullptr;
  a.s2w = infer ? op.d_s2w : nullptr;
  a.h16 = h16_mask(op, train_fwd);
  if (op.small_n) {
    a.by = op.fin_by; a.bx = op.fin_bx;
    if (op.fin && cm::conv_fin_ok(a)) return {CONV_FIN, form(op.d_wfin16, op.d_wfin, op.d_wfin_h2)};
    return {CONV_SMALLN, FORM_FP32};
  }
  if (op.d_w1x1_16 && infer && cm::conv1x1_f16_ok(a, op.NB)) return {CONV_1X1_F16, FORM_F16};
  return {CONV_GENERIC, form(cm::conv_par_f16_variant(op.MB, op.NB, g.bz, g.by, g.bx) ? op.d_wfrag16 : nullptr, nullptr, nullptr)};
}

bool route_takes_h16(ConvRoute r, int mask) {
  switch (r.kernel) {
    case CONV_F16D: return true;
    case CONV_UPS: return r.form == FORM_F16 && !(mask & ~5);
    case CONV_FIRST: return !(mask & ~4);
    case CONV_FIN: case CONV_SMALLN: return !(mask & ~3);
    default: return false;
  }
}

int plan_h16(cm_model *m) {
  if (m->precision != CM_PRECISION_F16 || cm::diag_env("CM_NO_H16")) return 0;
  auto takes = [&](const Op &o, int role) { return route_takes_h16(conv_route(o, m->precision, false, false), role); };
  for (auto &ap : m->acts) {
    Act *a = ap.get();
    bool ok = false;
    for (const Op &o : m->ops)
      if (o.kind == OP_CONV && o.out_act == a && !o.skip_if_fused) ok = takes(o, 4);
    for (const Op &o : m->ops) {
      if (!ok) break;
      if (o.kind == OP_ATTNBLK && o.ab_x == a) ok = false;
      if (o.kind == OP_ATTN && (o.qkv == a->d || o.aout == a->d)) ok = false;
      if (o.kind != OP_CONV || o.skip_if_fused) continue;
      const int role = (o.in0 == a ? 1 : 0) | (o.in1 == a ? 2 : 0) | (o.resid_act == a ? 8 : 0) | (o.skip0 == a ? 16 : 0) | (o.skip1 == a ? 32 : 0);
      if (role) ok = takes(o, role);
    }
    a->h16 = ok;
  }
  return 0;
}

int plan_slot_consumers(cm_model *m) {
  if (cm::diag_env("CM_NO_SLOT_GN")) return 0;
  const int nops = (int)m->ops.size();
  for (int i = 0; i < nops; ++i) {
    Op &g = m->ops[i];
    if (g.kind != OP_GNFIN || g.qr_consumer || g.in_attn_block) continue;
    int ncons = 0, cons = -1;
    for (int j = 0; j < nops; ++j)
      if (m->ops[j].kind == OP_CONV && m->ops[j].gn_op == i) { ++ncons; cons = j; }
    if (ncons != 1) continue;
    const ConvRoute r = conv_route(m->ops[cons], m->precision, false, false);
    g.from_slots = r.kernel == CONV_WINO && r.form != FORM_FP32;
  }
  return 0;
}

int build_time_table(cm_model *m) {
  const cm_unet_config &c = m->cfg;
  const int te = c.base_channels, tx = c.base_channels * c.time_multiple;
  std::vector<float> Wd((size_t)m->nproj * tx), bd((size_t)m->nproj);
  int off = 0;
  auto visit = [&](const BlockDesc &b) {
    if (b.kind != 0) return;
    const Param &w = P(m, b.prefix + ".dense_1.weight");
    const Param &bb = P(m, b.prefix + ".dense_1.bias");
    std::copy(w.host.begin(), w.host.end(), Wd.begin() + (size_t)off * tx);
    std::copy(bb.host.begin(), bb.host.end(), bd.begin() + off);
    off += b.cout;
  };
  for (auto &b : m->enc) visit(b);
  for (auto &b : m->bott) visit(b);
  for (auto &b : m->dec) visit(b);
  float *dT, *dW1, *db1, *dW2, *db2, *dWd, *dbd;
  if (upload(m, P(m, "time_embeddings.time_blocks.0.weight").host, &dT)) return 1;
  if (upload(m, P(m, "time_embeddings.time_blocks.1.weight").host, &dW1)) return 1;
  if (upload(m, P(m, "time_embeddings.time_blocks.1.bias").host, &db1)) return 1;
  if (upload(m, P(m, "time_embeddings.time_blocks.3.weight").host, &dW2)) return 1;
  if (upload(m, P(m, "time_embeddings.time_blocks.3.bias").host, &db2)) return 1;
  if (upload(m, Wd, &dWd)) return 1;
  if (upload(m, bd, &dbd)) return 1;
  m->d_time[0] = dT; m->d_time[1] = dW1; m->d_time[2] = db1; m->d_time[3] = dW2; m->d_time[4] = db2;
  m->d_time[5] = dWd; m->d_time[6] = dbd;
  CM_HIP(cm::launch_time_mlp(dT, dW1, db1, dW2, db2, dWd, dbd, te, tx, m->nproj, TIME_ROWS, nullptr, m->temb_table, nullptr, m->stream));
  CM_HIP(hipStreamSynchronize(m->stream));
  return 0;
}

int run_combine(cm_model *m, cm::CombineArgs &cb, hipStream_t st);
struct Op;
static thread_local const Op *tl_fin_next = nullptr;
static thread_local int tl_fin_b0 = 0;
static thread_local bool tl_fin_done = false;

int run_gnfin(const Op &g, float *mr, int B, hipStream_t st, int b0) {
  const Act *g0 = g.g0, *g1 = g.g1;
  const int Ct = g0->C + (g1 ? g1->C : 0);
  CM_HIP(cm::launch_gn_finalize(g0->part + (size_t)b0 * g0->nslots * g0->C * 2, g0->cnt + (size_t)b0 * g0->nslots, g0->nslots, g0->C,
                                g1 ? g1->part + (size_t)b0 * g1->nslots * g1->C * 2 : nullptr, g1 ? g1->cnt + (size_t)b0 * g1->nslots : nullptr,
                                g1 ? g1->nslots : 0, g1 ? g1->C : 0, g0->V(), g.gamma, g.beta, GN_GROUPS, GN_EPS,
                                g.gn_out + (size_t)b0 * 2 * Ct, mr ? mr + (size_t)b0 * 2 * Ct : nullptr, B, st));
  return 0;
}

int run_conv_qr(cm_model *m, const Op &op, ConvForm form, int B, hipStream_t st, int b0) {
  const Op &gop = m->ops[op.gn_op];
  const Act *g0 = gop.g0, *g1 = gop.g1;
  const cm::ConvArgs &ca = op.ca;
  const size_t V = (size_t)ca.Zo * ca.Yo * ca.Xo;
  cm::QrArgs q{};
  q.src0 = ca.src0 + (size_t)b0 * V * ca.C0; q.C0 = ca.C0;
  q.src1 = ca.src1 ? ca.src1 + (size_t)b0 * V * ca.C1 : nullptr; q.C1 = ca.C1;
  q.part0 = g0->part + (size_t)b0 * g0->nslots * g0->C * 2; q.cnt0 = g0->cnt + (size_t)b0 * g0->nslots; q.ns0 = g0->nslots;
  if (g1) { q.part1 = g1->part + (size_t)b0 * g1->nslots * g1->C * 2; q.cnt1 = g1->cnt + (size_t)b0 * g1->nslots; q.ns1 = g1->nslots; }
  if (g0->C != ca.C0 || (g1 ? g1->C : 0) != ca.C1) return fail("quarter-resolution conv %s: statistics and sources disagree", op.label.c_str());
  q.gamma = gop.gamma; q.beta = gop.beta; q.groups = GN_GROUPS; q.eps = GN_EPS; q.silu = ca.silu;
  if (op.dbg_raw) { q.gamma = q.beta = nullptr; q.raw = 1; q.silu = 0; }
  q.wq = op.d_wqr; q.bias = ca.bias;
  q.wq6 = op.d_wqr_b6;
  q.three = form == FORM_B3 ? 1 : 0;
  if (form == FORM_H2) { q.wq6 = op.d_wqr_h2; q.three = 2; q.h2_oscale = op.h2_oscale; }
  q.temb = ca.temb; q.temb_stride = ca.temb_stride; q.tidx = ca.tidx + b0;
  q.resid = ca.resid ? ca.resid + (size_t)b0 * V * ca.res_cs : nullptr; q.res_cs = ca.res_cs;
  if (m->train_fwd) {
    if (op.pm_off >= 0) { q.pm = m->dropmask + (size_t)b0 * m->nproj + op.pm_off; q.pm_stride = m->nproj; }
    if (m->use_train_temb && op.temb_off >= 0) { q.temb = m->train_temb + op.temb_off; q.tidx = m->train_iota + b0; }
  } else if (op.d_wqr_skip) {
    q.s2w = op.d_wqr_skip;
    q.s2src0 = op.skip0->d + (size_t)b0 * V * op.skip0->C; q.s2C0 = op.skip0->C;
    q.s2src1 = op.skip1 ? op.skip1->d + (size_t)b0 * V * op.skip1->C : nullptr; q.s2C1 = op.skip1 ? op.skip1->C : 0;
    q.resid = nullptr;
    q.bias = op.d_bias_fused;
  }
  q.out = ca.out + (size_t)b0 * V * ca.out_cs; q.out_cs = ca.out_cs; q.Co = ca.Co; q.B = B; q.Y = ca.Yo; q.X = ca.Xo;
  const int ns = ca.Yo * ca.Xo > 32 ? 4 : 2;
  q.stat_C = op.stat_act->C;
  q.stat_part = op.stat_act->part + (size_t)b0 * ns * q.stat_C * 2;
  q.stat_cnt = op.stat_act->cnt + (size_t)b0 * ns;
  op.stat_act->nslots = ns;
  op.prof_B = B;
  if (m->train_fwd && !cm::conv_qr2_b6_ok(q)) return fail("quarter-resolution conv %s: no six-term form for the training forward", op.label.c_str());
  CM_HIP(cm::launch_conv_qr(q, st));
  return 0;
}

int run_conv(cm_model *m, const Op &op, int B, hipStream_t st, int b0, int slab) {
  const ConvRoute route = conv_route(op, m->precision, m->train_fwd, m->h2_stale, op.in0 && op.in0->part && op.in0->nslots > 0);
  if (route.kernel == CONV_NONE) return 0;
  if (route.kernel == CONV_QR) return run_conv_qr(m, op, route.form, B, st, b0);
  cm::ConvArgs ca = op.ca;
  ca.B = B;
  op.prof_B = B;
  ca.nts = (B + ca.bs - 1) / ca.bs;
  const size_t Vs = (size_t)ca.Zs * ca.Ys * ca.Xs, Vo = (size_t)ca.Zo * ca.Yo * ca.Xo;
  ca.h16 = h16_mask(op, m->train_fwd);
  auto adv = [&](const float *p, size_t elems, int bit) { return p + ((ca.h16 & bit) ? elems / 2 : elems); };
  ca.src0 = adv(ca.src0, (size_t)b0 * Vs * ca.C0, 1);
  if (ca.src1) ca.src1 = adv(ca.src1, (size_t)b0 * Vs * ca.C1, 2);
  if (ca.gn) ca.gn += (size_t)b0 * 2 * (ca.C0 + ca.C1);
  ca.tidx += b0;
  if (m->train_fwd && op.pm_off >= 0) { ca.pm = m->dropmask + (size_t)b0 * m->nproj + op.pm_off; ca.pm_stride = m->nproj; }
  if (m->use_train_temb && op.temb_off >= 0) { ca.temb = m->train_temb + op.temb_off; ca.tidx = m->train_iota + b0; }
  if (ca.resid) ca.resid = adv(ca.resid, (size_t)b0 * Vo * ca.res_cs, 8);
  if (op.d_s2w && !m->train_fwd) {
    if (!op.wino && 32 * op.MB > cm::conv_halo_voxels(ca)) return fail("fused skip conv: tile rows exceed the staged box");
    ca.s2w = op.d_s2w;
    ca.s2src0 = adv(op.skip0->d, (size_t)b0 * Vo * op.skip0->C, 16); ca.s2C0 = op.skip0->C;
    ca.s2src1 = op.skip1 ? adv(op.skip1->d, (size_t)b0 * Vo * op.skip1->C, 32) : nullptr; ca.s2C1 = op.skip1 ? op.skip1->C : 0;
    ca.resid = nullptr;
    ca.bias = op.d_bias_fused;
  }
  ca.out = const_cast<float *>(adv(ca.out, (size_t)b0 * Vo * ca.out_cs, 4));
  if (ca.h16 && !route_takes_h16(route, ca.h16))
    return fail("conv %s: f16 tensors (mask %d) reach a kernel without f16 tensor support", op.label.c_str(), ca.h16);
  auto stat_slots = [&](int ns) -> int {
    if (!op.stat_act) return 0;
    if (ns > MAX_SLOTS) return fail("statistics slots %d exceed %d", ns, MAX_SLOTS);
    ca.stat_C = op.stat_act->C;
    ca.stat_ns = ns;
    ca.stat_part = op.stat_act->part + (size_t)b0 * ns * ca.stat_C * 2;
    ca.stat_cnt = op.stat_act->cnt + (size_t)b0 * ns;
    return 0;
  };
  const int ns_tile = ca.ntz * ca.nty * ca.ntx * op.MB * (ca.par ? 8 : 1);
  if (stat_slots(ns_tile)) return 1;
  switch (route.kernel) {
    case CONV_NONE: case CONV_QR: break;
    case CONV_KSPLIT: {
      cm::ConvArgs ka = ca;
      const int V = op.out_act->V();
      float *scratch = m->ks_scratch + (size_t)slab * m->ks_scratch_floats;
      ka.temb = nullptr; ka.resid = nullptr; ka.stat_part = nullptr; ka.bias = op.d_zero_bias;
      ka.out = scratch; ka.out_cs = ka.Co;
      ka.ks = op.ks; ka.kpart = (long long)B * V * ka.Co;
      CM_HIP(cm::launch_conv(ka, op.MB, op.NB, st));
      cm::CombineArgs cb{};
      cb.part = scratch; cb.S = op.ks; cb.stride = ka.kpart;
      cb.bias = ca.bias; cb.temb = ca.temb; cb.temb_stride = ca.temb_stride; cb.tidx = ca.tidx;
      cb.resid = ca.resid; cb.res_cs = ca.res_cs;
      cb.out = ca.out; cb.C = ka.Co; cb.V = V; cb.B = B;
      cb.nslots = (V + 31) / 32;
      cb.stat_part = op.stat_act->part + (size_t)b0 * cb.nslots * cb.C * 2;
      cb.stat_cnt = op.stat_act->cnt + (size_t)b0 * cb.nslots;
      op.stat_act->nslots = cb.nslots;
      return run_combine(m, cb, st);
    }
    case CONV_UPS:
      if (route.form == FORM_F16) { ca.wfrag = op.d_wups16; ca.wpar_stride = op.wups16_stride; }
      else if (route.form != FORM_FP32) { ca.wfrag = op.d_wups_b6; ca.wpar_stride = op.wups_b6_stride; }
      ca.f16 = route.form;
      if (route.form == FORM_H2) {
        const Act *si = op.in0;
        ca.wfrag = op.d_wups_h2; ca.h2_oscale = op.h2_oscale;
        ca.gp0 = si->part + (size_t)b0 * si->nslots * si->C * 2; ca.gc0 = si->cnt + (size_t)b0 * si->nslots; ca.gns0 = si->nslots;
      }
      ca.bz = op.ups_tz; ca.by = op.ups_ty; ca.bx = op.ups_tx;
      ca.ntz = ca.Zs / ca.bz; ca.nty = ca.Ys / ca.by; ca.ntx = ca.Xs / ca.bx;
      if (stat_slots(cm::conv_ups_slots(ca, op.ups_mbw))) return 1;
      if (op.stat_act) op.stat_act->nslots = ca.stat_ns;
      CM_HIP(cm::launch_conv_ups(ca, op.ups_mbw, op.ups_planes, op.NB, st));
      break;
    case CONV_F16D:
      ca.bz = op.f16d_bz; ca.by = op.f16d_by; ca.bx = op.f16d_bx;
      ca.wfrag = op.d_w16d;
      if (ca.s2w) ca.s2w = op.d_w16d_skip;
      if (stat_slots(cm::conv_f16d_slots(ca, op.f16d_mbw))) return 1;
      if (op.stat_act) op.stat_act->nslots = ca.stat_ns;
      CM_HIP(cm::launch_conv_f16d(ca, op.f16d_mbw, st));
      break;
    case CONV_WINO: {
      const bool f16 = route.form == FORM_F16;
      ca.wfrag = f16 ? op.d_wwino16 : route.form == FORM_H2 ? op.d_wwino_h2 : route.form == FORM_FP32 ? op.d_wwino : op.d_wwino_b6;
      if (!f16) ca.f16 = route.form;
      if (route.form == FORM_H2) ca.h2_oscale = op.h2_oscale;
      if (ca.gn && op.gn_op >= 0 && m->ops[op.gn_op].fin_skipped[slab & 3] && !m->train_fwd) {
        const Op &g = m->ops[op.gn_op];
        const Act *g0 = g.g0, *g1 = g.g1;
        if (cm::conv_wino_p_taken(ca, f16, true)) {
          ca.gp0 = g0->part + (size_t)b0 * g0->nslots * g0->C * 2; ca.gc0 = g0->cnt + (size_t)b0 * g0->nslots; ca.gns0 = g0->nslots;
          if (g1) { ca.gp1 = g1->part + (size_t)b0 * g1->nslots * g1->C * 2; ca.gc1 = g1->cnt + (size_t)b0 * g1->nslots; ca.gns1 = g1->nslots; }
          ca.gs_gamma = g.gamma; ca.gs_beta = g.beta; ca.gs_groups = GN_GROUPS; ca.gs_eps = GN_EPS;
          ca.gn = nullptr;
        } else if (run_gnfin(g, nullptr, B, st, b0)) {
          return 1;
        }
      }
      if (op.stat_act) op.stat_act->nslots = ns_tile;
      CM_HIP(cm::launch_conv_wino(ca, f16, st));
      break;
    }
    case CONV_FIRST:
      if (op.stat_act) op.stat_act->nslots = ns_tile;
      CM_HIP(cm::launch_conv_first(ca, op.first_cin, op.d_wfirst, st));
      break;
    case CONV_FIN: {
      const ConvForm f = route.form;
      ca.by = op.fin_by; ca.bx = op.fin_bx;
      ca.h2_oscale = op.h2_oscale;
      CM_HIP(cm::launch_conv_fin(ca, f == FORM_F16 ? op.d_wfin16 : f == FORM_H2 ? op.d_wfin_h2 : op.d_wfin, f == FORM_F16 ? 1 : f == FORM_H2 ? 3 : f == FORM_B3 ? 2 : 0, st));
      break;
    }
    case CONV_SMALLN:
      CM_HIP(cm::launch_conv_smalln(ca, op.MB, op.d_wsmall, st));
      break;
    case CONV_1X1_F16:
      ca.wfrag = op.d_w1x1_16;
      CM_HIP(cm::launch_conv1x1_f16(ca, op.NB, st));
      break;
    case CONV_GENERIC:
      if (route.form == FORM_F16) { ca.wfrag = op.d_wfrag16; ca.wpar_stride = op.wpar_stride16; ca.f16 = 1; }
      if (op.stat_act) op.stat_act->nslots = ns_tile;
      CM_HIP(cm::launch_conv(ca, op.MB, op.NB, st));
      break;
  }
  return 0;
}

int run_combine(cm_model *m, cm::CombineArgs &cb, hipStream_t st) {
  static const bool no_fuse = cm::diag_env("CM_NO_FUSE_GNFIN") != nullptr;
  const Op *f = tl_fin_next;
  tl_fin_done = false;
  if (f && !no_fuse && (!f->g1 || f->g1->V() == cb.V)) {
    const Act *g1 = f->g1;
    const int b0 = tl_fin_b0, Ct = cb.C + (g1 ? g1->C : 0);
    cb.fin_gamma = f->gamma; cb.fin_beta = f->beta;
    cb.fin_gn = f->gn_out + (size_t)b0 * 2 * Ct;
    cb.fin_mr = f->gn_mr ? f->gn_mr + (size_t)b0 * 2 * Ct : nullptr;
    cb.fin_p1 = g1 ? g1->part + (size_t)b0 * g1->nslots * g1->C * 2 : nullptr;
    cb.fin_n1 = g1 ? g1->cnt + (size_t)b0 * g1->nslots : nullptr;
    cb.fin_ns1 = g1 ? g1->nslots : 0; cb.fin_C1 = g1 ? g1->C : 0;
    cb.fin_groups = GN_GROUPS; cb.fin_eps = GN_EPS;
    if (cm::combine_gn_ok(cb)) {
      CM_HIP(cm::launch_combine_gn(cb, st));
      tl_fin_done = true;
      return 0;
    }
  }
  CM_HIP(cm::launch_ksplit_combine(cb, st));
  return 0;
}

int run_ops(cm_model *m, int B, hipStream_t st, int b0 = 0, int slab = 0) {
  for (size_t oi = 0; oi < m->ops.size(); ++oi) {
    Op &op = m->ops[oi];
    if (op.kind == OP_ATTNBLK ? m->train_fwd : (op.in_attn_block && !m->train_fwd)) continue;
    hipEvent_t e0 = nullptr, e1 = nullptr;
    if (m->profile) {
      CM_HIP(hipEventCreate(&e0));
      CM_HIP(hipEventCreate(&e1));
      CM_HIP(hipEventRecord(e0, st));
    }
    {
      static const bool sync_ops = cm::diag_env("CM_SYNC_OPS") != nullptr;
      if (sync_ops) {
        const hipError_t e = hipDeviceSynchronize();
        fprintf(stderr, "[cm] forward reaches op %zu %s (%s)\n", oi, op.label.c_str(), hipGetErrorString(e));
        fflush(stderr);
      }
    }
    tl_fin_next = nullptr; tl_fin_done = false;
    size_t fin_at = 0;
    if ((op.kind == OP_CONV && op.ks > 1) || op.kind == OP_ATTNBLK) {
      const Act *produced = op.kind == OP_CONV ? op.out_act : op.ab_out;
      size_t j = oi + 1;
      while (j < m->ops.size() && (m->ops[j].kind == OP_ATTNBLK ? m->train_fwd : (m->ops[j].in_attn_block && !m->train_fwd))) ++j;
      if (j < m->ops.size() && m->ops[j].kind == OP_GNFIN && m->ops[j].g0 == produced && !(m->ops[j].qr_consumer && !m->train_fwd)) { tl_fin_next = &m->ops[j]; tl_fin_b0 = b0; fin_at = j; }
    }
    switch (op.kind) {
      case OP_CONV:
        if (run_conv(m, op, B, st, b0, slab)) return 1;
        break;
      case OP_STATS: {
        const Act *t = op.act;
        CM_HIP(cm::launch_chan_stats(t->d + (size_t)b0 * t->V() * t->C, B, t->V(), t->C, t->nslice,
                                     t->part + (size_t)b0 * t->nslice * t->C * 2, t->cnt + (size_t)b0 * t->nslice, st));
        const_cast<Act *>(t)->nslots = t->nslice;
        break;
      }
      case OP_GNFIN: {
        if (op.qr_consumer && !m->train_fwd) break;
        op.fin_skipped[slab & 3] = false;
        const auto few = [](const Act *t) { return t->nslots <= 16; };
        if (op.from_slots && !m->train_fwd && few(op.g0) && (!op.g1 || few(op.g1)) &&
            (!op.g1 || op.g1->V() == op.g0->V())) {
          op.fin_skipped[slab & 3] = true;
          break;
        }
        if (op.g1 && op.g1->V() != op.g0->V()) return fail("concat sources disagree on voxel count");
        if (run_gnfin(op, op.gn_mr, B, st, b0)) return 1;
        break;
      }
      case OP_ATTN:
        if (m->precision == CM_PRECISION_F16 && !m->train_fwd && op.E / ATTN_HEADS == 32 && !cm::diag_env("CM_NO_ATTN_F16"))
          CM_HIP(cm::launch_attn_core_f16(op.qkv + (size_t)b0 * op.S * 3 * op.E, op.aout + (size_t)b0 * op.S * op.E, B, op.S,
                                          op.E, ATTN_HEADS, st));
        else
          CM_HIP(cm::launch_attn_core(op.qkv + (size_t)b0 * op.S * 3 * op.E, op.aout + (size_t)b0 * op.S * op.E, B, op.S,
                                      op.E, ATTN_HEADS, st));
        break;
      case OP_ATTNBLK: {
        const Op &gop = m->ops[op.ab_gn], &qop = m->ops[op.ab_qkv], &oop = m->ops[op.ab_outc];
        float *scratch = m->ks_scratch + (size_t)slab * m->ks_scratch_floats;
        const size_t xoff = (size_t)b0 * op.S * op.E;
        cm::AttnBlockArgs aa{};
        aa.x = op.ab_x->d + xoff; aa.gamma = gop.gamma; aa.beta = gop.beta;
        aa.w_in = op.d_win; aa.b_in = qop.ca.bias; aa.w_out = op.d_wout;
        aa.part = scratch; aa.B = B; aa.S = op.S; aa.E = op.E; aa.heads = ATTN_HEADS; aa.groups = GN_GROUPS; aa.eps = GN_EPS;
        CM_HIP(cm::launch_attn_block(aa, st));
        cm::CombineArgs cb{};
        cb.part = scratch; cb.S = ATTN_HEADS; cb.stride = (long long)B * op.S * op.E;
        cb.bias = oop.ca.bias; cb.temb = nullptr; cb.tidx = m->tbuf;
        cb.resid = aa.x; cb.res_cs = op.E;
        cb.out = op.ab_out->d + xoff; cb.C = op.E; cb.V = op.S; cb.B = B;
        cb.nslots = (op.S + 31) / 32;
        cb.stat_part = op.ab_out->part + (size_t)b0 * cb.nslots * cb.C * 2;
        cb.stat_cnt = op.ab_out->cnt + (size_t)b0 * cb.nslots;
        op.ab_out->nslots = cb.nslots;
        if (run_combine(m, cb, st)) return 1;
        break;
      }
    }
    if (m->profile) {
      CM_HIP(hipEventRecord(e1, st));
      m->prof_events[slab & 3].push_back({(int)oi, {e0, e1}});
    }
    if (tl_fin_done) oi = fin_at;
    tl_fin_next = nullptr; tl_fin_done = false;
  }
  return 0;
}

int prof_begin(cm_model *m, hipStream_t st) {
  if (!m->profile) return 0;
  for (int i = 0; i < K_NCLASS; ++i) { m->prof_ms[i] = 0; m->prof_n[i] = 0; m->prof_union_ms[i] = 0; }
  for (Op &op : m->ops) { op.prof_ms = 0; op.prof_n = 0; }
  if (!m->prof_base) CM_HIP(hipEventCreate(&m->prof_base));
  CM_HIP(hipEventRecord(m->prof_base, st));
  return 0;
}

int prof_collect(cm_model *m, hipStream_t st) {
  if (!m->profile) return 0;
  CM_HIP(hipDeviceSynchronize());
  (void)st;
  std::vector<std::pair<float, float>> iv[K_NCLASS];
  for (int ln = 0; ln < 4; ++ln) {
    for (auto &pe : m->prof_events[ln]) {
      float t0 = 0, t1 = 0;
      CM_HIP(hipEventElapsedTime(&t0, m->prof_base, pe.second.first));
      CM_HIP(hipEventElapsedTime(&t1, m->prof_base, pe.second.second));
      const float ms = t1 - t0;
      Op &op = m->ops[pe.first];
      op.prof_ms += ms;
// ... 480 lines not shown
  if (s->T > TIME_ROWS) return fail("timesteps %d exceed the %d-row time-embedding table (embeddings.py:7)", s->T, TIME_ROWS);
  if (opts->sampler == CM_SAMPLER_FM_EULER && (opts->fm_steps < 1 || opts->fm_time_max_pos < 1 || opts->fm_time_max_pos > TIME_ROWS))
    return fail("flow-matching sampler needs fm_steps >= 1 and 1 <= fm_time_max_pos <= %d", TIME_ROWS);
  DevGuard g(m->device);
  hipStream_t st = stream ? (hipStream_t)stream : m->stream;
  const cm_unet_config &c = m->cfg;
  const size_t per = (size_t)m->per_sample();
  const std::vector<int> order = visit_order(s, opts);
  const bool mass = opts->guidance == CM_GUIDANCE_MASS_PRESERVATION && opts->sampler == CM_SAMPLER_DDPM;
  if (mass && c.in_channels < 3) return fail("mass_preservation guidance needs >= 3 channels (r, u, v), model has %d", c.in_channels);
  if (mass && !m->mass_q && dev_alloc(m, (void **)&m->mass_q, (size_t)c.max_batch * 3 * c.rows * c.cols * c.future_len * sizeof(float)))
    return 1;
  if (prof_begin(m, st)) return 1;
  if (d_xT) CM_HIP(hipMemcpyAsync(m->xstate, d_xT, B * per * sizeof(float), hipMemcpyDeviceToDevice, st));
  else CM_HIP(cm::launch_randn(m->xstate, B, (long long)per, opts->seed, opts->sample_id_base, 0x7fffffff, st));
  if (d_history) CM_HIP(hipMemcpyAsync(d_history, m->xstate, B * per * sizeof(float), hipMemcpyDeviceToDevice, st));
  CM_HIP(cm::launch_assemble_input(d_past, m->xstate, m->x8, B, c.in_channels, c.rows, c.cols, c.past_len, c.future_len, 3, st));

  const int last = s->T - 1;
  float beta_t = s->tab[CM_TAB_BETA][last], sab_t = s->tab[CM_TAB_SQRT_ALPHA_BAR][last],
        s1m_t = s->tab[CM_TAB_SQRT_ONE_MINUS_ALPHA_BAR][last];
  static const int want_lanes = getenv("CM_LANES") ? atoi(getenv("CM_LANES")) : 2;
  int lanes = std::max(1, std::min(4, want_lanes));
  if (B < 8 * lanes || stream || opts->use_graph) lanes = 1;
  static const bool prof_lanes = getenv("CM_PROFILE_LANES") != nullptr;
  if (m->profile && !prof_lanes) lanes = 1;
  int Bl[4], off[4];
  hipStream_t sts[4] = {st, m->lane_stream[1], m->lane_stream[2], m->lane_stream[3]};
  for (int ln = 0, o = 0; ln < lanes; ++ln) {
    Bl[ln] = B / lanes + (ln < B % lanes ? 1 : 0);
    off[ln] = o;
    o += Bl[ln];
  }
  if (lanes > 1) {
    CM_HIP(hipEventRecord(m->ev_fork, st));
    for (int ln = 1; ln < lanes; ++ln) CM_HIP(hipStreamWaitEvent(sts[ln], m->ev_fork, 0));
  }
  std::vector<cm::StepRow> rows(order.size());
  for (size_t k = 0; k < order.size(); ++k) {
    const int t = order[k];
    cm::StepRow &r = rows[k];
    r.t = t; r.step = t; r.mass = 0.f;
    if (opts->sampler == CM_SAMPLER_FM_EULER) {
      r.c_x = 1.0f; r.c_eps = (float)(1.0 / (double)opts->fm_steps); r.c_noise = 0.f;
      r.draw = 0; r.guid = 0.f;
      r.step = (int)k;
    } else if (opts->sampler == CM_SAMPLER_DDIM) {
      const float sab_p = s->tab[CM_TAB_SQRT_ALPHA_BAR][t], s1m_p = s->tab[CM_TAB_SQRT_ONE_MINUS_ALPHA_BAR][t];
      const float sig = opts->ddim_sigma;
      r.c_x = sab_p / sab_t;
      r.c_eps = sqrtf(1.0f - sab_p * sab_p - sig * sig) - sab_p * s1m_t / sab_t;
      r.c_noise = sig;
      r.draw = 1;
      r.guid = opts->guidance == CM_GUIDANCE_SPARSITY ? opts->lambda_guidance * sqrtf(beta_t) : 0.f;
      beta_t = s->tab[CM_TAB_BETA][t]; sab_t = sab_p; s1m_t = s1m_p;
    } else {
      ddpm_coeffs(s, t, &r.c_x, &r.c_eps, &r.c_noise);
      r.draw = t > 0;
      r.guid = opts->guidance == CM_GUIDANCE_SPARSITY ? opts->lambda_guidance * sqrtf(s->tab[CM_TAB_BETA][t]) : 0.f;
      if (mass) {
        const float a = 1.0f - s->tab[CM_TAB_BETA][t];
        r.mass = 1.0f - a;
      }
    }
  }
  auto base_args = [&]() {
    cm::StepArgs a{};
    a.C = c.in_channels; a.H = c.rows; a.W = c.cols; a.P = c.past_len; a.F = c.future_len;
    a.seed = opts->seed; a.cs = 8;
    return a;
  };
  const size_t per_q = (size_t)3 * c.rows * c.cols * c.future_len;
  auto mass_step = [&](int b0, int Bn, float cmass, float *hist, const cm::StepRow *tab, long long boff, hipStream_t ls) -> int {
    float *x = m->xstate + (size_t)b0 * per;
    float *q = m->mass_q + (size_t)b0 * per_q;
    CM_HIP(cm::launch_mass_grad(x, c.in_channels, q, 3, Bn, c.rows, c.cols, c.future_len, 1.0f, 1.0f, 0.1f, ls));
    cm::MassApplyArgs ma{};
    ma.x = x; ma.q = q; ma.x8 = m->x8 + (size_t)b0 * m->L() * c.rows * c.cols * 8; ma.hist = hist;
    ma.B = Bn; ma.C = c.in_channels; ma.H = c.rows; ma.W = c.cols; ma.P = c.past_len; ma.F = c.future_len;
    ma.c = cmass; ma.tab = tab; ma.kctr = m->d_kctr; ma.row_stride = (long long)B * per; ma.boff = boff;
    CM_HIP(cm::launch_mass_apply(ma, ls));
    return 0;
  };
  const bool graph = opts->use_graph && !m->profile && lanes == 1 && !stream && order.size() >= 3;
  if (graph) {
    if (m->steptab_cap < rows.size()) {
      if (dev_alloc(m, (void **)&m->d_steptab, rows.size() * sizeof(cm::StepRow))) return 1;
      m->steptab_cap = rows.size();
    }
    if (!m->d_kctr && dev_alloc(m, (void **)&m->d_kctr, sizeof(int))) return 1;
    CM_HIP(hipMemcpyAsync(m->d_steptab, rows.data(), rows.size() * sizeof(cm::StepRow), hipMemcpyHostToDevice, st));
    CM_HIP(hipMemsetAsync(m->d_kctr, 0xFF, sizeof(int), st));
    CM_HIP(hipStreamSynchronize(st));
    auto enqueue_step = [&]() -> int {
      CM_HIP(cm::launch_step_begin(m->tbuf, B, m->d_steptab, m->d_kctr, st));
      if (denoise(m, B, st, 0, 0)) return 1;
      cm::StepArgs al = base_args();
      al.B = B; al.x = m->xstate; al.eps_cl = m->eps_cl; al.x8 = m->x8;
      al.sample_id_base = opts->sample_id_base;
      al.tab = m->d_steptab; al.kctr = m->d_kctr; al.row_stride = (long long)B * per; al.boff = 0;
      al.hist = d_history; al.noise = d_noise;
      CM_HIP(cm::launch_sampler_step(al, st));
      if (mass && mass_step(0, B, 0.f, d_history, m->d_steptab, 0, st)) return 1;
      return 0;
    };
    if (enqueue_step()) return 1;
    hipGraph_t g = nullptr;
    hipGraphExec_t ge = nullptr;
    CM_HIP(hipStreamBeginCapture(st, hipStreamCaptureModeRelaxed));
    const int rc_cap = enqueue_step();
    hipError_t ec = hipStreamEndCapture(st, &g);
    if (rc_cap || ec != hipSuccess) { if (g) hipGraphDestroy(g); return rc_cap ? 1 : fail("graph capture failed: %s", hipGetErrorString(ec)); }
    ec = hipGraphInstantiate(&ge, g, nullptr, nullptr, 0);
    if (ec != hipSuccess) { hipGraphDestroy(g); return fail("graph instantiate failed: %s", hipGetErrorString(ec)); }
    for (size_t k = 1; k < order.size() && ec == hipSuccess; ++k) ec = hipGraphLaunch(ge, st);
    if (ec == hipSuccess) ec = hipStreamSynchronize(st);
    hipGraphExecDestroy(ge);
    hipGraphDestroy(g);
    if (ec != hipSuccess) return fail("graph replay failed: %s", hipGetErrorString(ec));
  }
  auto lane_steps = [&](int ln, size_t k0, size_t k1) -> int {
    const int b0 = off[ln], Bn = Bl[ln];
    hipStream_t ls = sts[ln];
    for (size_t k = k0; k < k1; ++k) {
      const int t = order[k];
      cm::StepArgs al = base_args();
      const cm::StepRow &r = rows[k];
      al.step = r.step; al.c_x = r.c_x; al.c_eps = r.c_eps; al.c_noise = r.c_noise; al.draw = r.draw; al.guid = r.guid;
      if (k == 0) CM_HIP(cm::launch_fill_t(m->tbuf + b0, Bn, t, ls));
      if (denoise(m, Bn, ls, b0, ln)) return 1;
      al.B = Bn;
      if (k + 1 < order.size()) { al.t_next = m->tbuf + b0; al.t_next_v = order[k + 1]; }
      al.x = m->xstate + (size_t)b0 * per;
      al.eps_cl = m->eps_cl + (size_t)b0 * m->L() * c.rows * c.cols * 8;
      al.x8 = m->x8 + (size_t)b0 * m->L() * c.rows * c.cols * 8;
      al.sample_id_base = opts->sample_id_base + b0;
      al.hist = d_history ? d_history + (k + 1) * B * per + (size_t)b0 * per : nullptr;
      al.noise = (d_noise && al.draw) ? d_noise + k * B * per + (size_t)b0 * per : nullptr;
      CM_HIP(cm::launch_sampler_step(al, ls));
      if (mass && mass_step(b0, Bn, r.mass, al.hist, nullptr, 0, ls)) return 1;
    }
    return 0;
  };
  if (!graph && lanes == 1) {
    if (lane_steps(0, 0, order.size())) return 1;
  } else if (!graph) {
    for (int ln = 0; ln < lanes; ++ln)
      if (lane_steps(ln, 0, 1)) return 1;
    std::vector<int> rcs((size_t)lanes, 0);
    std::vector<std::string> errs((size_t)lanes);
    std::vector<std::thread> workers;
    std::vector<char> started((size_t)lanes, 0);
    try {
      workers.reserve((size_t)lanes);
      for (int ln = 1; ln < lanes; ++ln) {
        try {
          workers.emplace_back([&, ln]() {
            try {
              if (hipSetDevice(m->device) != hipSuccess) { rcs[ln] = 1; errs[ln] = "hipSetDevice failed in a lane thread"; return; }
              rcs[ln] = lane_steps(ln, 1, order.size());
              if (rcs[ln]) errs[ln] = g_err;
            } catch (const std::exception &e) {
              rcs[ln] = 1;
              try { errs[ln] = e.what(); } catch (...) {}
            } catch (...) {
              rcs[ln] = 1;
            }
          });
          started[ln] = 1;
        } catch (...) {
          started[ln] = 0;
        }
      }
      rcs[0] = lane_steps(0, 1, order.size());
      if (rcs[0]) errs[0] = g_err;
      for (int ln = 1; ln < lanes; ++ln)
        if (!started[ln]) {
          rcs[ln] = lane_steps(ln, 1, order.size());
          if (rcs[ln]) errs[ln] = g_err;
        }
    } catch (const std::exception &e) {
      rcs[0] = 1;
      try { errs[0] = e.what(); } catch (...) {}
    } catch (...) {
      rcs[0] = 1;
    }
    for (auto &w : workers) w.join();
    for (int ln = 0; ln < lanes; ++ln)
      if (rcs[ln]) return fail("lane %d: %s", ln, errs[ln].empty() ? "exception in the lane's enqueue thread" : errs[ln].c_str());
  }
  for (int ln = 1; ln < lanes; ++ln) {
    CM_HIP(hipEventRecord(m->ev_join[ln], sts[ln]));
    CM_HIP(hipStreamWaitEvent(st, m->ev_join[ln], 0));
  }
  CM_HIP(hipMemcpyAsync(d_out, m->xstate, B * per * sizeof(float), hipMemcpyDeviceToDevice, st));
  if (opts->check_finite) {
    if (!m->d_nonfinite && dev_alloc(m, (void **)&m->d_nonfinite, sizeof(int))) return 1;
    CM_HIP(cm::launch_count_nonfinite(m->xstate, (long long)(B * per), m->d_nonfinite, st));
    int bad = 0;
    CM_HIP(hipMemcpyAsync(&bad, m->d_nonfinite, sizeof(int), hipMemcpyDeviceToHost, st));
    CM_HIP(hipStreamSynchronize(st));
    if (prof_collect(m, st)) return 1;
    if (bad) return fail("sampling produced %d non-finite values out of %lld (check_finite)", bad, (long long)(B * per));
    return 0;
  }
  return prof_collect(m, st);
}

int cm_sample_loop_host(cm_model *m, const cm_schedule *s, const float *h_past, const float *h_xT, const float *h_noise,
                        const cm_sample_opts *opts, float *h_out, float *h_history, int32_t B) {
  if (check_ready(m, B)) return 1;
  if (!s || !h_past || !opts || !h_out) return fail("null argument");
  DevGuard g(m->device);
  const cm_unet_config &c = m->cfg;
  const size_t per = (size_t)m->per_sample();
  const size_t per_past = (size_t)c.in_channels * c.rows * c.cols * c.past_len;
  const size_t nsteps = visit_order(s, opts).size();
  CM_HIP(hipMemcpy(m->stage_past, h_past, B * per_past * sizeof(float), hipMemcpyHostToDevice));
  if (h_xT) CM_HIP(hipMemcpy(m->stage_fut, h_xT, B * per * sizeof(float), hipMemcpyHostToDevice));
  float *dn = nullptr, *dh = nullptr;
  if (h_noise) {
    CM_HIP(hipMalloc((void **)&dn, nsteps * B * per * sizeof(float)));
// ... 56 lines not shown
  }
  double wbytes = 0;
  for (const Param &p : m->params) wbytes += 4.0 * p.numel();
  if (flops) *flops = f;
  if (bytes) *bytes = by + wbytes;
  return 0;
}

int cm_profile_report(cm_model *m, char *buf, int64_t capacity) {
  CM_NOT_DIT(m, "cm_profile_report");
  if (!m || !buf || capacity < 1) return fail("null argument");
  std::string out;
  char line[512];
  for (const Op &op : m->ops) {
    if (op.prof_n == 0) continue;
    const double us = op.prof_ms * 1e3 / op.prof_n;
    if (op.kind == OP_CONV) {
      const cm::ConvArgs &a = op.ca;
      const double tf = op.flops_per_sample * op.prof_B / (us * 1e-6) / 1e12;
      snprintf(line, sizeof(line), "%-52s %9.1f us %7.2f TF %8.1f MF/sample B%d ks%d  %s%d NB%d box %dx%dx%dx%d grid %dx%d CK%d lds %zu\n", op.label.c_str(), us, tf,
               op.flops_per_sample / 1e6, op.prof_B, op.ks,
               "MB", op.MB, op.NB, a.bs, a.bz, a.by, a.bx, a.nts * a.ntz * a.nty * a.ntx,
               (a.Co + 32 * op.NB - 1) / (32 * op.NB), a.CK, cm::conv_lds_bytes(a, op.MB, op.NB));
    } else {
      snprintf(line, sizeof(line), "%-52s %9.1f us\n", op.label.c_str(), us);
    }
    out += line;
  }
  snprintf(buf, (size_t)capacity, "%s", out.c_str());
  return 0;
}

int cm_frame_metrics(int32_t device, const float *d_pred, const float *d_gt, int32_t N, int32_t Cc, int32_t H, int32_t W,
                     int32_t F, double *h_out, float *h_minmax) {
  if (!d_pred || !d_gt || !h_out || !h_minmax) return fail("null argument");
  if (N < 1 || Cc < 1 || H < 1 || W < 1 || F < 1) return fail("bad shape");
  DevGuard g(device);
  const size_t cells = (size_t)N * Cc * F;
  double *d_out = nullptr;
  float *d_mm = nullptr;
  CM_HIP(hipMalloc((void **)&d_out, cells * 8 * sizeof(double)));
  hipError_t e = hipMalloc((void **)&d_mm, cells * 2 * sizeof(float));
  if (e == hipSuccess) e = cm::launch_frame_metrics(d_pred, d_gt, N, Cc, H, W, F, d_out, d_mm, nullptr);
  if (e == hipSuccess) e = hipDeviceSynchronize();
  if (e == hipSuccess) e = hipMemcpy(h_out, d_out, cells * 8 * sizeof(double), hipMemcpyDeviceToHost);
  if (e == hipSuccess) e = hipMemcpy(h_minmax, d_mm, cells * 2 * sizeof(float), hipMemcpyDeviceToHost);
  hipFree(d_out);
  if (d_mm) hipFree(d_mm);
  if (e != hipSuccess) return fail("frame metrics failed: %s", hipGetErrorString(e));
  return 0;
}

int cm_mass_preservation_grad(int32_t device, const float *d_x, int32_t B, int32_t Cc, int32_t H, int32_t W, int32_t L,
                              float delta_t, float delta_l, float eps, float *d_grad, void *stream) {
  if (!d_x || !d_grad) return fail("null argument");
  if (B < 1 || H < 1 || W < 1 || L < 1) return fail("bad shape [%d,%d,%d,%d,%d]", B, Cc, H, W, L);
  if (Cc < 3) return fail("mass_preservation gradient needs >= 3 channels (r, u, v: guidance.py:25-31), got %d", Cc);
  if (delta_t == 0.f || delta_l == 0.f) return fail("delta_t and delta_l must be non-zero");
  if (d_x == d_grad) return fail("d_grad must not alias d_x (the gradient is written out of place)");
  DevGuard g(device);
  CM_HIP(cm::launch_mass_grad(d_x, Cc, d_grad, Cc, B, H, W, L, delta_t, delta_l, eps, (hipStream_t)stream));
  return 0;
}

int cm_debug_conv_flags(int32_t flags) {
  cm::conv_dbg_override = flags;
  return 0;
}

int cm_debug_conv_count(const cm_model *m, int32_t *count) {
  CM_NOT_DIT(m, "cm_debug_conv_count");
  if (!m || !m->finalized || !count) return fail("model not finalized");
  *count = (int32_t)m->ops.size();
  return 0;
}

int cm_debug_conv_info(const cm_model *m, int32_t index, char *buf, int64_t capacity) {
  CM_NOT_DIT(m, "cm_debug_conv_info");
  if (!m || !m->finalized || !buf || index < 0 || index >= (int)m->ops.size()) return fail("bad argument");
  const Op &op = m->ops[index];
  if (op.kind != OP_CONV) { snprintf(buf, (size_t)capacity, "other %s", op.label.c_str()); return 0; }
  const cm::ConvArgs &a = op.ca;
  const ConvRoute r = conv_route(op, m->precision, false, m->h2_stale);
  snprintf(buf, (size_t)capacity, "conv %s %d %d %d %d %d %d %d %d %d %d %d %d %d %d %d %d %d %d %d %s %d", op.label.c_str(), a.ntaps, a.stride, a.par,
           a.C0 + a.C1, a.Co, a.Zo, a.Yo, a.Xo, op.NB, op.MB, a.bz, a.by, a.bx, op.ks,
           (op.small_n ? 1 : 0) | (op.first_k ? 2 : 0) | (op.stat_act ? 4 : 0) | (op.skip_if_fused ? 8 : 0) | (a.CK == 32 ? 16 : 0),
           op.out_act ? op.out_act->C : a.Co,
           a.C0, a.C1, op.wino ? 1 : 0,
           kConvKernelName[r.kernel], (int)r.form);
  return 0;
}

int cm_debug_conv_io(cm_model *m, int32_t index, int32_t mode, const float *h_in0, const float *h_in1, float *h_out, int32_t B) {
  CM_NOT_DIT(m, "cm_debug_conv_io");
  if (check_ready(m, B)) return 1;
  if (!h_in0 || !h_out || index < 0 || index >= (int)m->ops.size()) return fail("bad argument");
  Op &op = m->ops[index];
  if (op.kind != OP_CONV || !op.in0 || !op.out_act) return fail("op %d is not a convolution", index);
  if ((op.in1 != nullptr) != (h_in1 != nullptr)) return fail("op %d has %d source tensors", index, op.in1 ? 2 : 1);
  DevGuard g(m->device);
  hipStream_t st = m->stream;
  const size_t Vs = (size_t)op.in0->V(), Vo = (size_t)op.out_act->V();
  CM_HIP(hipMemcpy(op.in0->d, h_in0, (size_t)B * Vs * op.in0->C * sizeof(float), hipMemcpyHostToDevice));
  if (op.in1) CM_HIP(hipMemcpy(op.in1->d, h_in1, (size_t)B * Vs * op.in1->C * sizeof(float), hipMemcpyHostToDevice));
  if (mode < 0 || mode > 3) return fail("mode %d", mode);
  Op tmp = op;
  if (mode != 3) {
    tmp.ca.gn = nullptr; tmp.ca.silu = 0; tmp.ca.temb = nullptr; tmp.temb_off = -1; tmp.ca.resid = nullptr; tmp.resid_act = nullptr;
    tmp.d_s2w = nullptr; tmp.d_wqr_skip = nullptr; tmp.dbg_raw = true; tmp.pm_off = -1;
    if (!tmp.qr) tmp.gn_op = -1;
  }
  tmp.skip_if_fused = false;
  tmp.dbg_h2 = mode == 2;
  if (mode == 1) { tmp.d_wwino_b6 = nullptr; tmp.d_wqr_b6 = nullptr; tmp.d_wups_b6 = nullptr; }
  const int ns_keep = op.stat_act ? op.stat_act->nslots : 0;
  const int ns_in_keep = op.in0->nslots;
  if (mode == 2 && op.ups && op.in0->part) {
    const Act *t = op.in0;
    CM_HIP(cm::launch_chan_stats(t->d, B, t->V(), t->C, t->nslice, t->part, t->cnt, st));
    const_cast<Act *>(t)->nslots = t->nslice;
  }
  const int rc = run_conv(m, tmp, B, st, 0, 0);
  const hipError_t e = hipStreamSynchronize(st);
  if (op.stat_act) op.stat_act->nslots = ns_keep;
  const_cast<Act *>(op.in0)->nslots = ns_in_keep;
  if (rc) return 1;
  if (e != hipSuccess) return fail("debug conv launch failed: %s", hipGetErrorString(e));
  CM_HIP(hipMemcpy(h_out, op.out_act->d, (size_t)B * Vo * op.out_act->C * sizeof(float), hipMemcpyDeviceToHost));
  return 0;
}

int cm_debug_wino_form_counts(int64_t counts[16], int32_t reset) {
  if (!counts) return fail("bad argument");
  long long c[16];
  cm::conv_wino_form_counts(c, reset != 0);
  for (int i = 0; i < 16; ++i) counts[i] = (int64_t)c[i];
  return 0;
}

int cm_debug_conv_stats(cm_model *m, int32_t index, int32_t B, float *h_part, float *h_cnt, int32_t *nslots, int32_t *C) {
  CM_NOT_DIT(m, "cm_debug_conv_stats");
  if (check_ready(m, B)) return 1;
  if (!nslots || !C || index < 0 || index >= (int)m->ops.size()) return fail("bad argument");
  const Op &op = m->ops[index];
  if (op.kind != OP_CONV || !op.stat_act || !op.stat_act->part) return fail("op %d writes no statistics", index);
  const Act *t = op.stat_act;
  *nslots = t->nslots;
  *C = t->C;
  DevGuard g(m->device);
  CM_HIP(hipStreamSynchronize(m->stream));
  if (h_part) CM_HIP(hipMemcpy(h_part, t->part, (size_t)B * t->nslots * t->C * 2 * sizeof(float), hipMemcpyDeviceToHost));
  if (h_cnt) CM_HIP(hipMemcpy(h_cnt, t->cnt, (size_t)B * t->nslots * sizeof(float), hipMemcpyDeviceToHost));
  return 0;
}

int cm_debug_time_conv(cm_model *m, int32_t index, int32_t MB, int32_t bz, int32_t by, int32_t bx, int32_t B,
                       int32_t iters, float *us) {
  CM_NOT_DIT(m, "cm_debug_time_conv");
  if (check_ready(m, B)) return 1;
  if (!us || index < 0 || index >= (int)m->ops.size() || iters < 1) return fail("bad argument");
  Op &op = m->ops[index];
  if (op.kind != OP_CONV || ((op.first_k || op.wino) && MB > 0)) return fail("op %d is not a tunable convolution", index);
  DevGuard g(m->device);
  hipStream_t st = m->stream;
  const Op saved = op;
  int rc = 0;
  if (MB > 0) {
    cm::ConvArgs &a = op.ca;
    const int osd = a.par ? 2 : 1;
    if (bz < 1 || by < 1 || bx < 1 || (bz * by * bx + 31) / 32 != MB || !cm::conv_variant_exists(MB, op.NB)) rc = fail("invalid geometry");
    if (!rc) {
      a.bs = 1; a.bz = bz; a.by = by; a.bx = bx;
// ... 106 lines not shown
```

Baseline: 928.6 denoise-steps/s, aggregate over 1 GPU under weak scaling (every GPU advances its own batch of 64 chains per step).

## Trim constant past-frame work in first/last convs and fuse sampler update into last conv

```diff
diff --git a/crowdmod-ddpm-4d_amd/csrc/cm_conv_fin.hip b/crowdmod-ddpm-4d_amd/csrc/cm_conv_fin.hip
--- a/crowdmod-ddpm-4d_amd/csrc/cm_conv_fin.hip
+++ b/crowdmod-ddpm-4d_amd/csrc/cm_conv_fin.hip
@@ -17,8 +17,8 @@
 constexpr int FIN_ROWS = 64;
 constexpr int FIN_PCOLS = 132;
 
-template <int MODE>
-__global__ __launch_bounds__(256, 2) void conv_fin_kernel(const ConvArgs a, const float *__restrict__ wfin, int ntx) {
+template <int MODE, int FUSE>
+__global__ __launch_bounds__(256, 2) void conv_fin_kernel(const ConvArgs a, const float *__restrict__ wfin, int ntx, const StepArgs sa_in) {
   constexpr bool F16 = MODE == 1, H2 = MODE == 3;
   constexpr int U0 = MODE >= 2 ? 3 : 0, NTW = MODE >= 2 ? 2 : 3;
   constexpr int NTM = F16 ? 1 : 3;
@@ -27,6 +27,9 @@
   float *A = lds;
   float *P = A + 4 * FIN_ROWS * RW;
   float *OACC = P + FIN_ROWS * FIN_PCOLS;
+  float *EPSB = OACC + 3 * 64 * 4;
+  StepArgs sa = sa_in;
+  if constexpr (FUSE != 0) cm_step_resolve(sa);
   const int tid = threadIdx.x, lane = tid & 63;
   const int wave = __builtin_amdgcn_readfirstlane(tid >> 6);
   const int r = lane & 31, hh = lane >> 5;
@@ -117,12 +120,15 @@
   for (int i = tid; i < 3 * 64 * 4; i += 256) OACC[i] = 0.f;
 
   const int Z = a.Zs;
+  const int zf = a.zo_first, ze = a.zo_end > 0 ? a.zo_end : a.Zo;
+  int zs, zl;
+  conv_fin_zloop(zf, ze, Z, &zs, &zl);
   constexpr int TA[6] = {0, 2, 1, 0, 1, 0}, TB[6] = {2, 0, 1, 1, 0, 0};
-  issue(0);
+  issue(zs);
   stage();
-  if (Z > 1) issue(1);
+  if (zs + 1 < zl) issue(zs + 1);
   __syncthreads();
-  for (int z = 0; z < Z; ++z) {
+  for (int z = zs; z < zl; ++z) {
     f32x16 acc[2];
 #pragma unroll
     for (int j = 0; j < 2; ++j)
@@ -158,13 +164,13 @@
         *reinterpret_cast<f32x4 *>(P + (size_t)(32 * j + r) * FIN_PCOLS + 4 * (8 * wave + 2 * g + hh)) = pv;
       }
     __syncthreads();
-    if (z + 1 < Z) {
+    if (z + 1 < zl) {
       stage();
-      if (z + 2 < Z) issue(z + 2);
+      if (z + 2 < zl) issue(z + 2);
     }
     if (gath) {
       const int zo = z + 1 - dzg;
-      if (zo >= 0 && zo < a.Zo) {
+      if (zo >= zf && zo < ze) {
         f32x4 s4 = {0.f, 0.f, 0.f, 0.f};
 #pragma unroll
         for (int t9 = 0; t9 < 9; ++t9) {
@@ -175,11 +181,20 @@
         f32x4 v = *reinterpret_cast<const f32x4 *>(oa) + s4;
         const bool last = dzg == 2 || (dzg == 1 && z == Z - 1);
         if (last) {
-          if (oin) {
-            float *o = a.out + ((size_t)((b * a.Zo + zo) * a.Yo + oy) * a.Xo + ox) * a.out_cs;
-#pragma unroll
-            for (int c = 0; c < 4; ++c)
-              if (c < a.Co) o[c] = v[c] + bias4[c];
+          if constexpr (FUSE == 1) {
+            *reinterpret_cast<f32x4 *>(EPSB + (size_t)((zo - zf) * 64 + gu) * 4) = v + bias4;
+          } else if (oin) {
+            if constexpr (FUSE == 2) {
+              const size_t cl = ((size_t)(b * a.Zo + zo) * a.Yo + oy) * a.Xo + ox;
+#pragma unroll
+              for (int c = 0; c < 4; ++c)
+                if (c < a.Co) cm_sampler_update(sa, b, ((long long)(c * sa.H + oy) * sa.W + ox) * sa.F + (zo - zf), c, cl, v[c] + bias4[c]);
+            } else {
+              float *o = a.out + ((size_t)((b * a.Zo + zo) * a.Yo + oy) * a.Xo + ox) * a.out_cs;
+#pragma unroll
+              for (int c = 0; c < 4; ++c)
+                if (c < a.Co) o[c] = v[c] + bias4[c];
+            }
           }
           v = f32x4{0.f, 0.f, 0.f, 0.f};
         }
@@ -187,6 +202,23 @@
       }
     }
     __syncthreads();
+  }
+  if constexpr (FUSE != 0) {
+    if (blockIdx.x == 0 && sa.t_next)
+      for (int i = tid; i < a.B; i += 256) sa.t_next[i] = sa.t_next_v;
+  }
+  if constexpr (FUSE == 1) {
+    const int nz = ze - zf, total = a.Co * NV * nz;
+    for (int idx = tid; idx < total; idx += 256) {
+      const int f = idx % nz;
+      int qv = idx / nz;
+      const int ux = qv % BX; qv /= BX;
+      const int uy = qv % BY;
+      const int c = qv / BY;
+      const int hy = y0 + uy, wx = x0 + ux;
+      const size_t cl = ((size_t)(b * a.Zo + zf + f) * a.Yo + hy) * a.Xo + wx;
+      cm_sampler_update(sa, b, ((long long)(c * sa.H + hy) * sa.W + wx) * sa.F + f, c, cl, EPSB[(size_t)(f * 64 + uy * BX + ux) * 4 + c]);
+    }
   }
 }
 
@@ -209,33 +241,48 @@
          a.bx > 0 && a.Yo % a.by == 0 && a.Xo % a.bx == 0 && (a.by + 2) * (a.bx + 2) <= FIN_ROWS && a.by * a.bx <= 64 && !(a.h16 & ~1);
 }
 
-size_t conv_fin_lds(bool f16) {
-  return ((size_t)2 * 2 * FIN_ROWS * (f16 ? 4 : 12) + (size_t)FIN_ROWS * FIN_PCOLS + 3 * 64 * 4) * sizeof(float);
-}
-
-hipError_t launch_conv_fin(const ConvArgs &a_in, const float *wfin, int mode, hipStream_t st) {
+size_t conv_fin_lds(bool f16, int fused_planes = 0) {
+  return ((size_t)2 * 2 * FIN_ROWS * (f16 ? 4 : 12) + (size_t)FIN_ROWS * FIN_PCOLS + 3 * 64 * 4 + (size_t)fused_planes * 64 * 4) * sizeof(float);
+}
+
+bool conv_fin_fuse_ok(const ConvArgs &a, const StepArgs &s) {
+  const int nz = a.zo_end - a.zo_first;
+  return conv_fin_ok(a) && s.x && a.zo_first == s.P && nz == s.F && nz >= 1 && nz <= 8 && a.Zo == s.P + s.F && a.Yo == s.H && a.Xo == s.W &&
+         a.Co == s.C && a.B == s.B && s.cs == a.out_cs;
+}
+
+template <int FUSE>
+static const void *conv_fin_fn(int mode) {
+  return mode == 1 ? reinterpret_cast<const void *>(conv_fin_kernel<1, FUSE>)
+       : mode == 2 ? reinterpret_cast<const void *>(conv_fin_kernel<2, FUSE>)
+       : mode == 3 ? reinterpret_cast<const void *>(conv_fin_kernel<3, FUSE>) : reinterpret_cast<const void *>(conv_fin_kernel<0, FUSE>);
+}
+
+hipError_t launch_conv_fin(const ConvArgs &a_in, const float *wfin, int mode, hipStream_t st, const StepArgs *step, int variant) {
   ConvArgs a = a_in;
   a.dbg = conv_dbg_flags();
   if (!conv_fin_ok(a) || mode < 0 || mode > 3) return hipErrorInvalidValue;
+  if (a.zo_end == 0 && a.zo_first == 0) a.zo_end = a.Zo;
+  if (a.zo_first < 0 || a.zo_end <= a.zo_first || a.zo_end > a.Zo) return hipErrorInvalidValue;
+  const int fuse = step ? (variant == 2 ? 2 : 1) : 0;
+  if (fuse && !conv_fin_fuse_ok(a, *step)) return hipErrorInvalidValue;
   const int nty = a.Yo / a.by, ntx = a.Xo / a.bx;
   a.nty = nty;
   const dim3 grid((unsigned)(a.B * nty * ntx));
-  const size_t lds = conv_fin_lds(mode == 1);
-  static bool attr_set[64][4] = {{false}};
+  const size_t lds = conv_fin_lds(mode == 1, fuse == 1 ? a.zo_end - a.zo_first : 0);
+  static bool attr_set[64][4][3] = {{{false}}};
   int dev = 0;
   (void)hipGetDevice(&dev);
-  const void *fn = mode == 1 ? reinterpret_cast<const void *>(conv_fin_kernel<1>)
-                 : mode == 2 ? reinterpret_cast<const void *>(conv_fin_kernel<2>)
-                 : mode == 3 ? reinterpret_cast<const void *>(conv_fin_kernel<3>) : reinterpret_cast<const void *>(conv_fin_kernel<0>);
-  if (!attr_set[dev & 63][mode]) {
+  const void *fn = fuse == 1 ? conv_fin_fn<1>(mode) : fuse == 2 ? conv_fin_fn<2>(mode) : conv_fin_fn<0>(mode);
+  if (!attr_set[dev & 63][mode][fuse]) {
     hipError_t e = hipFuncSetAttribute(fn, hipFuncAttributeMaxDynamicSharedMemorySize, 160 * 1024);
     if (e != hipSuccess) return e;
-    attr_set[dev & 63][mode] = true;
-  }
-  if (mode == 1) hipLaunchKernelGGL(conv_fin_kernel<1>, grid, dim3(256), lds, st, a, wfin, ntx);
-  else if (mode == 2) hipLaunchKernelGGL(conv_fin_kernel<2>, grid, dim3(256), lds, st, a, wfin, ntx);
-  else if (mode == 3) hipLaunchKernelGGL(conv_fin_kernel<3>, grid, dim3(256), lds, st, a, wfin, ntx);
-  else hipLaunchKernelGGL(conv_fin_kernel<0>, grid, dim3(256), lds, st, a, wfin, ntx);
+    attr_set[dev & 63][mode][fuse] = true;
+  }
+  const StepArgs sa = step ? *step : StepArgs{};
+  void *params[] = {(void *)&a, (void *)&wfin, (void *)&ntx, (void *)&sa};
+  hipError_t e = hipLaunchKernel(fn, grid, dim3(256), params, lds, st);
+  if (e != hipSuccess) return e;
   return hipGetLastError();
 }
 
diff --git a/crowdmod-ddpm-4d_amd/csrc/cm_conv_io.hip b/crowdmod-ddpm-4d_amd/csrc/cm_conv_io.hip
--- a/crowdmod-ddpm-4d_amd/csrc/cm_conv_io.hip
+++ b/crowdmod-ddpm-4d_amd/csrc/cm_conv_io.hip
@@ -16,9 +16,10 @@
   const int r = lane & 31, hh = lane >> 5;
   int tile = blockIdx.x;
   if (!(gridDim.x & 7) && !(a.dbg & 4096)) tile = (tile & 7) * (int)(gridDim.x >> 3) + (tile >> 3);
+  const int ntz_run = a.ntz - a.tz_first;
   const int ty = tile % a.nty; tile /= a.nty;
-  const int tz = tile % a.ntz;
-  const int b = tile / a.ntz;
+  const int tz = a.tz_first + tile % ntz_run;
+  const int b = tile / ntz_run;
   const int nt = blockIdx.y;
   const int X = a.Xo, bz = a.bz, by = a.by;
   const int z0 = tz * bz, y0 = ty * by;
@@ -158,9 +159,9 @@
 hipError_t launch_conv_first(const ConvArgs &a_in, int cin, const float *wpk, hipStream_t st) {
   ConvArgs a = a_in;
   a.dbg = conv_dbg_flags();
-  if (!conv_first_ok(a, cin)) return hipErrorInvalidValue;
+  if (!conv_first_ok(a, cin) || a.tz_first < 0 || a.tz_first >= a.ntz) return hipErrorInvalidValue;
   const int nblk = conv_first_blocks(a);
-  const dim3 grid((unsigned)(a.B * a.ntz * a.nty), (unsigned)((a.Co + 31) / 32));
+  const dim3 grid((unsigned)(a.B * (a.ntz - a.tz_first) * a.nty), (unsigned)((a.Co + 31) / 32));
   const size_t lds = conv_first_lds(a, cin);
   if (cin == 4) hipLaunchKernelGGL(conv_first_kernel<4>, grid, dim3(256), lds, st, a, wpk, nblk);
   else hipLaunchKernelGGL(conv_first_kernel<8>, grid, dim3(256), lds, st, a, wpk, nblk);
diff --git a/crowdmod-ddpm-4d_amd/csrc/cm_dit_host.inc b/crowdmod-ddpm-4d_amd/csrc/cm_dit_host.inc
--- a/crowdmod-ddpm-4d_amd/csrc/cm_dit_host.inc
+++ b/crowdmod-ddpm-4d_amd/csrc/cm_dit_host.inc
@@ -195,8 +195,8 @@
   return 0;
 }
 
-int denoise(cm_model *m, int B, hipStream_t st, int b0, int slab) {
-  return m->dit ? dit_forward(m, B, st, b0) : run_ops(m, B, st, b0, slab);
+int denoise(cm_model *m, int B, hipStream_t st, int b0, int slab, const LoopEnds *le = nullptr) {
+  return m->dit ? dit_forward(m, B, st, b0) : run_ops(m, B, st, b0, slab, le);
 }
 
 }
diff --git a/crowdmod-ddpm-4d_amd/csrc/cm_host_selftest.cpp b/crowdmod-ddpm-4d_amd/csrc/cm_host_selftest.cpp
--- a/crowdmod-ddpm-4d_amd/csrc/cm_host_selftest.cpp
+++ b/crowdmod-ddpm-4d_amd/csrc/cm_host_selftest.cpp
@@ -461,6 +461,85 @@
   printf("test_conv_route: %d combinations walked\n", walked);
 }
 
+void test_loop_ends() {
+  struct G { int Y, X, bz, by; };
+  const G grids[] = {{12, 36, 4, 3}, {28, 24, 4, 4}, {24, 72, 2, 3}, {13, 37, 1, 13}, {11, 35, 1, 11}};
+  for (const G &g : grids) {
+    Op op = route_class_op(RC_FIRST, CM_PRECISION_F32);
+    op.ca.Zo = op.ca.Zs = 8; op.ca.Yo = op.ca.Ys = g.Y; op.ca.Xo = op.ca.Xs = g.X;
+    pick_tile_first(op);
+    EXPECT(op.ca.bz == g.bz && op.ca.by == g.by && op.ca.ntz == 8 / g.bz);
+    const int t = cm::conv_first_const_ztiles(op.ca.bz, op.ca.ntz, 5);
+    EXPECT(t == 4 / g.bz && 2 * t == op.ca.ntz);
+    for (int tz = 0; tz < op.ca.ntz; ++tz) EXPECT((tz < t) == (tz * g.bz + g.bz <= 4));
+  }
+  for (int P = 1; P <= 9; ++P)
+    for (int F = 1; F <= 4; ++F)
+      for (int bz = 1; bz <= P + F; ++bz) {
+        if ((P + F) % bz) continue;
+        const int ntz = (P + F) / bz, t = cm::conv_first_const_ztiles(bz, ntz, P);
+        EXPECT(t >= 0 && t < ntz && t * bz <= P - 1);
+        EXPECT(((P - 1) % bz == 0 && P > 1) ? t == (P - 1) / bz : t == 0);
+      }
+  EXPECT(cm::conv_first_const_ztiles(4, 2, 1) == 0 && cm::conv_first_const_ztiles(1, 2, 1) == 0 && cm::conv_first_const_ztiles(3, 3, 5) == 0);
+  for (int P = 1; P <= 6; ++P)
+    for (int F = 1; F <= 4; ++F) {
+      const int Z = P + F;
+      int zs, zl;
+      cm::conv_fin_zloop(P, Z, Z, &zs, &zl);
+      EXPECT(zs == P - 1 && zl == Z);
+      cm::conv_fin_zloop(0, Z, Z, &zs, &zl);
+      EXPECT(zs == 0 && zl == Z);
+      cm::conv_fin_zloop(0, 1, Z, &zs, &zl);
+      EXPECT(zs == 0 && zl == 2);
+    }
+  {
+    static float x8, eps;
+    std::vector<Op> ops;
+    ops.push_back(route_class_op(RC_FIRST, CM_PRECISION_F32));
+    ops.push_back(route_class_op(RC_WINO_FULL, CM_PRECISION_F32));
+    ops.push_back(route_class_op(RC_LAST, CM_PRECISION_F32));
+    ops[0].ca.src0 = &x8; pick_tile_first(ops[0]);
+    ops[2].ca.out = &eps;
+    LoopEnds le = loop_ends_plan(ops, &x8, &eps, 7, CM_PRECISION_F32, false, 5, 3, 4, 4);
+    EXPECT(le.tz_first == 1 && le.zo_first == 5 && le.zo_end == 8 && le.fuse == 1);
+    le = loop_ends_plan(ops, &x8, &eps, 15, CM_PRECISION_F32, false, 5, 3, 4, 4);
+    EXPECT(le.fuse == 2);
+    le = loop_ends_plan(ops, &x8, &eps, 0, CM_PRECISION_F32, false, 5, 3, 4, 4);
+    EXPECT(le.tz_first == 0 && le.zo_end == 0 && le.fuse == 0);
+    le = loop_ends_plan(ops, &x8, &eps, 1, CM_PRECISION_F32, false, 5, 3, 4, 4);
+    EXPECT(le.tz_first == 0 && le.zo_first == 5 && le.zo_end == 8 && le.fuse == 0);
+    le = loop_ends_plan(ops, &x8, &eps, 4, CM_PRECISION_F32, false, 5, 3, 4, 4);
+    EXPECT(le.tz_first == 1 && le.zo_end == 0 && le.fuse == 0);
+    le = loop_ends_plan(ops, &x8, &eps, 7, CM_PRECISION_F32, false, 1, 7, 4, 4);
+    EXPECT(le.tz_first == 0 && le.zo_first == 1 && le.zo_end == 8 && le.fuse == 1);
+    le = loop_ends_plan(ops, &x8, &eps, 7, CM_PRECISION_F32, false, 7, 1, 4, 4);
+    EXPECT(le.tz_first == 0 && le.zo_first == 7 && le.zo_end == 8 && le.fuse == 1);
+    le = loop_ends_plan(ops, &x8, &eps, 7, CM_PRECISION_F32, false, 5, 3, 3, 4);
+    EXPECT(le.zo_end == 8 && le.fuse == 0);
+    ops[2].ca.C1 = 32;
+    le = loop_ends_plan(ops, &x8, &eps, 7, CM_PRECISION_F32, false, 5, 3, 4, 4);
+    EXPECT(le.tz_first == 1 && le.zo_end == 0 && le.fuse == 0);
+    ops[0].first_k = false;
+    le = loop_ends_plan(ops, &x8, &eps, 7, CM_PRECISION_F32, false, 5, 3, 4, 4);
+    EXPECT(le.tz_first == 0);
+  }
+  {
+    Op op = route_class_op(RC_LAST, CM_PRECISION_F32);
+    cm::ConvArgs a = op.ca;
+    a.by = op.fin_by; a.bx = op.fin_bx; a.B = 2; a.zo_first = 5; a.zo_end = 8;
+    static float x;
+    cm::StepArgs st{};
+    st.x = &x; st.B = 2; st.C = 4; st.H = 12; st.W = 36; st.P = 5; st.F = 3; st.cs = 8;
+    EXPECT(cm::conv_fin_fuse_ok(a, st));
+    st.F = 2; EXPECT(!cm::conv_fin_fuse_ok(a, st)); st.F = 3;
+    st.C = 3; EXPECT(!cm::conv_fin_fuse_ok(a, st)); st.C = 4;
+    a.zo_first = 4; EXPECT(!cm::conv_fin_fuse_ok(a, st)); a.zo_first = 5;
+    st.B = 1; EXPECT(!cm::conv_fin_fuse_ok(a, st));
+  }
+  printf("test_loop_ends ok\n");
+}
+
 void test_misc_errors() {
   EXPECT(cm_abi_version() == CM_ABI_VERSION);
   EXPECT(cm_device_count(nullptr) != 0);
@@ -486,6 +565,7 @@
   test_round3_packers();
   test_wino_form_dispatch();
   test_conv_route();
+  test_loop_ends();
   test_misc_errors();
   printf("selftest ok: %d checks\n", g_checks);
   return 0;
diff --git a/crowdmod-ddpm-4d_amd/csrc/cm_kernels.h b/crowdmod-ddpm-4d_amd/csrc/cm_kernels.h
--- a/crowdmod-ddpm-4d_amd/csrc/cm_kernels.h
+++ b/crowdmod-ddpm-4d_amd/csrc/cm_kernels.h
@@ -92,7 +92,10 @@
   int zsplit;
   int h16;
   float h2_oscale;
-  alignas(8) unsigned char layout_pad[40];
+  alignas(8) int zo_first;
+  int zo_end;
+  int tz_first;
+  unsigned char layout_pad[28];
   const float *gs_gamma, *gs_beta;
   int gs_groups;
   float gs_eps;
@@ -265,7 +268,15 @@
 
 bool conv_fin_pick(int Y, int X, int *by, int *bx);
 bool conv_fin_ok(const ConvArgs &a);
-hipError_t launch_conv_fin(const ConvArgs &a, const float *wfin, int mode , hipStream_t st);
+struct StepArgs;
+bool conv_fin_fuse_ok(const ConvArgs &a, const StepArgs &s);
+hipError_t launch_conv_fin(const ConvArgs &a, const float *wfin, int mode , hipStream_t st,
+                           const StepArgs *step = nullptr, int variant = 1);
+inline int conv_first_const_ztiles(int bz, int ntz, int P) {
+  if (bz < 1 || P < 2 || (P - 1) % bz) return 0;
+  const int n = (P - 1) / bz;
+  return n < ntz ? n : 0;
+}
 hipError_t launch_fin_pack(const float *w_ref , float *wfin, int Co, int mode , hipStream_t st, float wscale = 1.f);
 constexpr size_t CM_FIN_W_FLOATS = 4 * 2 * 3 * 64 * 4;
 
@@ -357,6 +368,64 @@
   long long *t_next; long long t_next_v;
 };
 hipError_t launch_sampler_step(const StepArgs &a, hipStream_t st);
+#ifdef __HIPCC__
+__device__ __forceinline__ void philox4x32_10(unsigned c0, unsigned c1, unsigned c2, unsigned c3, unsigned k0,
+                                              unsigned k1, unsigned out[4]) {
+#pragma unroll
+  for (int i = 0; i < 10; ++i) {
+    const unsigned long long p0 = 0xD2511F53ull * c0;
+    const unsigned long long p1 = 0xCD9E8D57ull * c2;
+    const unsigned n0 = (unsigned)(p1 >> 32) ^ c1 ^ k0;
+    const unsigned n1 = (unsigned)p1;
+    const unsigned n2 = (unsigned)(p0 >> 32) ^ c3 ^ k1;
+    const unsigned n3 = (unsigned)p0;
+    c0 = n0; c1 = n1; c2 = n2; c3 = n3;
+    k0 += 0x9E3779B9u;
+    k1 += 0xBB67AE85u;
+  }
+  out[0] = c0; out[1] = c1; out[2] = c2; out[3] = c3;
+}
+
+__device__ __forceinline__ float philox_normal(unsigned long long seed, long long sample, int step, long long elem) {
+  unsigned r[4];
+  philox4x32_10((unsigned)(elem >> 1), (unsigned)sample, (unsigned)step, (unsigned)((sample >> 32) ^ 0x5eed),
+                (unsigned)seed, (unsigned)(seed >> 32), r);
+  const float u1 = ((float)(r[0] >> 8) + 0.5f) * (1.0f / 16777216.0f);
+  const float u2 = ((float)(r[1] >> 8) + 0.5f) * (1.0f / 16777216.0f);
+  const float rad = sqrtf(-2.0f * __logf(u1));
+  const float ang = 6.283185307179586f * u2;
+  return (elem & 1) ? rad * __sinf(ang) : rad * __cosf(ang);
+}
+
+__device__ __forceinline__ void cm_step_resolve(StepArgs &a) {
+  if (a.tab) {
+    const int k = *a.kctr;
+    const StepRow r = a.tab[k];
+    a.c_x = r.c_x; a.c_eps = r.c_eps; a.c_noise = r.c_noise; a.guid = r.guid; a.draw = r.draw; a.step = r.step;
+    if (a.noise) a.noise += (long long)k * a.row_stride + a.boff;
+    if (a.hist) a.hist += (long long)(k + 1) * a.row_stride + a.boff;
+  }
+}
+__device__ __forceinline__ void cm_sampler_update(const StepArgs &a, long long b, long long e, int c, size_t cl, float eps) {
+  const long long i = b * ((long long)a.C * a.H * a.W * a.F) + e;
+  float z = 0.f;
+  if (a.draw) z = a.noise ? a.noise[i] : philox_normal(a.seed, a.sample_id_base + b, a.step, e);
+  float xn;
+  {
+#pragma clang fp contract(off)
+    const float pe = a.c_eps * eps, pz = a.c_noise * z;
+    xn = pz + __builtin_fmaf(a.c_x, a.x[i], pe);
+    if (a.guid != 0.f && c == 0) xn = xn - a.guid * (xn > 0.f ? 1.f : (xn < 0.f ? -1.f : 0.f));
+  }
+  a.x[i] = xn;
+  if (a.x8) a.x8[cl * 8 + c] = xn;
+  if (a.hist) a.hist[i] = xn;
+}
+#endif
+__host__ __device__ inline void conv_fin_zloop(int zf, int ze, int Z, int *zs, int *zl) {
+  *zs = zf > 0 ? zf - 1 : 0;
+  *zl = ze < Z ? ze + 1 : Z;
+}
 hipError_t launch_mass_grad(const float *x, int Cin, float *q, int Cout, int B, int H, int W, int L, float delta_t,
                             float delta_l, float eps, hipStream_t st);
 struct MassApplyArgs {
diff --git a/crowdmod-ddpm-4d_amd/csrc/cm_misc.hip b/crowdmod-ddpm-4d_amd/csrc/cm_misc.hip
--- a/crowdmod-ddpm-4d_amd/csrc/cm_misc.hip
+++ b/crowdmod-ddpm-4d_amd/csrc/cm_misc.hip
@@ -763,34 +763,6 @@
   return hipGetLastError();
 }
 
-__device__ __forceinline__ void philox4x32_10(unsigned c0, unsigned c1, unsigned c2, unsigned c3, unsigned k0,
-                                              unsigned k1, unsigned out[4]) {
-#pragma unroll
-  for (int i = 0; i < 10; ++i) {
-    const unsigned long long p0 = 0xD2511F53ull * c0;
-    const unsigned long long p1 = 0xCD9E8D57ull * c2;
-    const unsigned n0 = (unsigned)(p1 >> 32) ^ c1 ^ k0;
-    const unsigned n1 = (unsigned)p1;
-    const unsigned n2 = (unsigned)(p0 >> 32) ^ c3 ^ k1;
-    const unsigned n3 = (unsigned)p0;
-    c0 = n0; c1 = n1; c2 = n2; c3 = n3;
-    k0 += 0x9E3779B9u;
-    k1 += 0xBB67AE85u;
-  }
-  out[0] = c0; out[1] = c1; out[2] = c2; out[3] = c3;
-}
-
-__device__ __forceinline__ float philox_normal(unsigned long long seed, long long sample, int step, long long elem) {
-  unsigned r[4];
-  philox4x32_10((unsigned)(elem >> 1), (unsigned)sample, (unsigned)step, (unsigned)((sample >> 32) ^ 0x5eed),
-                (unsigned)seed, (unsigned)(seed >> 32), r);
-  const float u1 = ((float)(r[0] >> 8) + 0.5f) * (1.0f / 16777216.0f);
-  const float u2 = ((float)(r[1] >> 8) + 0.5f) * (1.0f / 16777216.0f);
-  const float rad = sqrtf(-2.0f * __logf(u1));
-  const float ang = 6.283185307179586f * u2;
-  return (elem & 1) ? rad * __sinf(ang) : rad * __cosf(ang);
-}
-
 __global__ __launch_bounds__(256) void randn_kernel(float *__restrict__ x, long long per, long long total,
                                                     unsigned long long seed, long long sample_id_base, int step) {
   const long long i = (long long)blockIdx.x * 256 + threadIdx.x;
@@ -808,13 +780,7 @@
 }
 
 __global__ __launch_bounds__(256) void sampler_step_kernel(StepArgs a) {
-  if (a.tab) {
-    const int k = *a.kctr;
-    const StepRow r = a.tab[k];
-    a.c_x = r.c_x; a.c_eps = r.c_eps; a.c_noise = r.c_noise; a.guid = r.guid; a.draw = r.draw; a.step = r.step;
-    if (a.noise) a.noise += (long long)k * a.row_stride + a.boff;
-    if (a.hist) a.hist += (long long)(k + 1) * a.row_stride + a.boff;
-  }
+  cm_step_resolve(a);
   const long long per = (long long)a.C * a.H * a.W * a.F;
   const long long total = per * a.B;
   const long long i = (long long)blockIdx.x * 256 + threadIdx.x;
@@ -828,14 +794,7 @@
   const int c = (int)(q / a.H);
   const int L = a.P + a.F;
   const size_t cl = ((((size_t)b * L + (a.P + f)) * a.H + hh) * a.W + w);
-  const float eps = a.eps_cl[cl * a.cs + c];
-  float z = 0.f;
-  if (a.draw) z = a.noise ? a.noise[i] : philox_normal(a.seed, a.sample_id_base + b, a.step, e);
-  float xn = a.c_x * a.x[i] + a.c_eps * eps + a.c_noise * z;
-  if (a.guid != 0.f && c == 0) xn -= a.guid * (xn > 0.f ? 1.f : (xn < 0.f ? -1.f : 0.f));
-  a.x[i] = xn;
-  if (a.x8) a.x8[cl * 8 + c] = xn;
-  if (a.hist) a.hist[i] = xn;
+  cm_sampler_update(a, b, e, c, cl, a.eps_cl[cl * a.cs + c]);
 }
 
 hipError_t launch_sampler_step(const StepArgs &a, hipStream_t st) {
diff --git a/crowdmod-ddpm-4d_amd/csrc/cm_model.cpp b/crowdmod-ddpm-4d_amd/csrc/cm_model.cpp
--- a/crowdmod-ddpm-4d_amd/csrc/cm_model.cpp
+++ b/crowdmod-ddpm-4d_amd/csrc/cm_model.cpp
@@ -213,6 +213,7 @@
   size_t steptab_cap = 0;
   int *d_kctr = nullptr;
   int *d_nonfinite = nullptr;
+  int loop_ends = cm::diag_env("CM_LOOP_ENDS") ? (atoi(cm::diag_env("CM_LOOP_ENDS")) & 15) : 7;
   float *mass_q = nullptr;
   float *stage_past = nullptr, *stage_fut = nullptr, *stage_out = nullptr;
   float *stage_noise = nullptr;
@@ -1413,6 +1414,27 @@
   }
 }
 
+struct LoopEnds {
+  int tz_first = 0;
+  int zo_first = 0, zo_end = 0;
+  int fuse = 0;
+  const cm::StepArgs *step = nullptr;
+};
+LoopEnds loop_ends_plan(const std::vector<Op> &ops, const float *x8, const float *eps_cl, int mask, int precision, bool h2_stale, int P, int F,
+                        int Cin, int Cout) {
+  LoopEnds le;
+  for (const Op &op : ops) {
+    if (op.kind != OP_CONV) continue;
+    const ConvRoute r = conv_route(op, precision, false, h2_stale);
+    if (r.kernel == CONV_FIRST && op.ca.src0 == x8 && (mask & 4)) le.tz_first = cm::conv_first_const_ztiles(op.ca.bz, op.ca.ntz, P);
+    if (r.kernel == CONV_FIN && op.ca.out == eps_cl && op.ca.Zo == P + F && (mask & 3)) {
+      le.zo_first = P; le.zo_end = P + F;
+      if ((mask & 2) && Cin == Cout && op.ca.Co == Cout && op.ca.out_cs == 8 && F <= 8) le.fuse = (mask & 8) ? 2 : 1;
+    }
+  }
+  return le;
+}
+
 int plan_h16(cm_model *m) {
   if (m->precision != CM_PRECISION_F16 || cm::diag_env("CM_NO_H16")) return 0;
   auto takes = [&](const Op &o, int role) { return route_takes_h16(conv_route(o, m->precision, false, false), role); };
@@ -1538,7 +1560,7 @@
   return 0;
 }
 
-int run_conv(cm_model *m, const Op &op, int B, hipStream_t st, int b0, int slab) {
+int run_conv(cm_model *m, const Op &op, int B, hipStream_t st, int b0, int slab, const LoopEnds *le = nullptr) {
   const ConvRoute route = conv_route(op, m->precision, m->train_fwd, m->h2_stale, op.in0 && op.in0->part && op.in0->nslots > 0);
   if (route.kernel == CONV_NONE) return 0;
   if (route.kernel == CONV_QR) return run_conv_qr(m, op, route.form, B, st, b0);
@@ -1645,13 +1667,17 @@
     }
     case CONV_FIRST:
       if (op.stat_act) op.stat_act->nslots = ns_tile;
+      if (le && op.ca.src0 == m->x8) ca.tz_first = le->tz_first;
       CM_HIP(cm::launch_conv_first(ca, op.first_cin, op.d_wfirst, st));
       break;
     case CONV_FIN: {
       const ConvForm f = route.form;
       ca.by = op.fin_by; ca.bx = op.fin_bx;
       ca.h2_oscale = op.h2_oscale;
-      CM_HIP(cm::launch_conv_fin(ca, f == FORM_F16 ? op.d_wfin16 : f == FORM_H2 ? op.d_wfin_h2 : op.d_wfin, f == FORM_F16 ? 1 : f == FORM_H2 ? 3 : f == FORM_B3 ? 2 : 0, st));
+      const bool ends = le && le->zo_end && op.ca.out == m->eps_cl;
+      if (ends) { ca.zo_first = le->zo_first; ca.zo_end = le->zo_end; }
+      CM_HIP(cm::launch_conv_fin(ca, f == FORM_F16 ? op.d_wfin16 : f == FORM_H2 ? op.d_wfin_h2 : op.d_wfin, f == FORM_F16 ? 1 : f == FORM_H2 ? 3 : f == FORM_B3 ? 2 : 0, st,
+                                 ends && le->fuse ? le->step : nullptr, ends ? le->fuse : 0));
       break;
     }
     case CONV_SMALLN:
@@ -1694,7 +1720,7 @@
   return 0;
 }
 
-int run_ops(cm_model *m, int B, hipStream_t st, int b0 = 0, int slab = 0) {
+int run_ops(cm_model *m, int B, hipStream_t st, int b0 = 0, int slab = 0, const LoopEnds *le = nullptr) {
   for (size_t oi = 0; oi < m->ops.size(); ++oi) {
     Op &op = m->ops[oi];
     if (op.kind == OP_ATTNBLK ? m->train_fwd : (op.in_attn_block && !m->train_fwd)) continue;
@@ -1722,7 +1748,7 @@
     }
     switch (op.kind) {
       case OP_CONV:
-        if (run_conv(m, op, B, st, b0, slab)) return 1;
+        if (run_conv(m, op, B, st, b0, slab, le)) return 1;
         break;
       case OP_STATS: {
         const Act *t = op.act;
@@ -2369,6 +2395,8 @@
     CM_HIP(cm::launch_mass_apply(ma, ls));
     return 0;
   };
+  const LoopEnds ends = m->dit ? LoopEnds{} : loop_ends_plan(m->ops, m->x8, m->eps_cl, m->loop_ends, m->precision, m->h2_stale, c.past_len,
+                                                             c.future_len, c.in_channels, c.out_channels);
   const bool graph = opts->use_graph && !m->profile && lanes == 1 && !stream && order.size() >= 3;
   if (graph) {
     if (m->steptab_cap < rows.size()) {
@@ -2379,23 +2407,26 @@
     CM_HIP(hipMemcpyAsync(m->d_steptab, rows.data(), rows.size() * sizeof(cm::StepRow), hipMemcpyHostToDevice, st));
     CM_HIP(hipMemsetAsync(m->d_kctr, 0xFF, sizeof(int), st));
     CM_HIP(hipStreamSynchronize(st));
-    auto enqueue_step = [&]() -> int {
+    auto enqueue_step = [&](bool first) -> int {
       CM_HIP(cm::launch_step_begin(m->tbuf, B, m->d_steptab, m->d_kctr, st));
-      if (denoise(m, B, st, 0, 0)) return 1;
       cm::StepArgs al = base_args();
       al.B = B; al.x = m->xstate; al.eps_cl = m->eps_cl; al.x8 = m->x8;
       al.sample_id_base = opts->sample_id_base;
       al.tab = m->d_steptab; al.kctr = m->d_kctr; al.row_stride = (long long)B * per; al.boff = 0;
       al.hist = d_history; al.noise = d_noise;
-      CM_HIP(cm::launch_sampler_step(al, st));
+      LoopEnds le = ends;
+      le.step = &al;
+      if (first) le.tz_first = 0;
+      if (denoise(m, B, st, 0, 0, &le)) return 1;
+      if (!ends.fuse) CM_HIP(cm::launch_sampler_step(al, st));
       if (mass && mass_step(0, B, 0.f, d_history, m->d_steptab, 0, st)) return 1;
       return 0;
     };
-    if (enqueue_step()) return 1;
+    if (enqueue_step(true)) return 1;
     hipGraph_t g = nullptr;
     hipGraphExec_t ge = nullptr;
     CM_HIP(hipStreamBeginCapture(st, hipStreamCaptureModeRelaxed));
-    const int rc_cap = enqueue_step();
+    const int rc_cap = enqueue_step(false);
     hipError_t ec = hipStreamEndCapture(st, &g);
     if (rc_cap || ec != hipSuccess) { if (g) hipGraphDestroy(g); return rc_cap ? 1 : fail("graph capture failed: %s", hipGetErrorString(ec)); }
     ec = hipGraphInstantiate(&ge, g, nullptr, nullptr, 0);
@@ -2415,7 +2446,6 @@
       const cm::StepRow &r = rows[k];
       al.step = r.step; al.c_x = r.c_x; al.c_eps = r.c_eps; al.c_noise = r.c_noise; al.draw = r.draw; al.guid = r.guid;
       if (k == 0) CM_HIP(cm::launch_fill_t(m->tbuf + b0, Bn, t, ls));
-      if (denoise(m, Bn, ls, b0, ln)) return 1;
       al.B = Bn;
       if (k + 1 < order.size()) { al.t_next = m->tbuf + b0; al.t_next_v = order[k + 1]; }
       al.x = m->xstate + (size_t)b0 * per;
@@ -2424,7 +2454,11 @@
       al.sample_id_base = opts->sample_id_base + b0;
       al.hist = d_history ? d_history + (k + 1) * B * per + (size_t)b0 * per : nullptr;
       al.noise = (d_noise && al.draw) ? d_noise + k * B * per + (size_t)b0 * per : nullptr;
-      CM_HIP(cm::launch_sampler_step(al, ls));
+      LoopEnds le = ends;
+      le.step = &al;
+      if (k == 0) le.tz_first = 0;
+      if (denoise(m, Bn, ls, b0, ln, &le)) return 1;
+      if (!ends.fuse) CM_HIP(cm::launch_sampler_step(al, ls));
       if (mass && mass_step(b0, Bn, r.mass, al.hist, nullptr, 0, ls)) return 1;
     }
     return 0;
@@ -2647,12 +2681,24 @@
   if (op.kind != OP_CONV) { snprintf(buf, (size_t)capacity, "other %s", op.label.c_str()); return 0; }
   const cm::ConvArgs &a = op.ca;
   const ConvRoute r = conv_route(op, m->precision, false, m->h2_stale);
-  snprintf(buf, (size_t)capacity, "conv %s %d %d %d %d %d %d %d %d %d %d %d %d %d %d %d %d %d %d %d %s %d", op.label.c_str(), a.ntaps, a.stride, a.par,
+  const LoopEnds le = loop_ends_plan(m->ops, m->x8, m->eps_cl, m->loop_ends, m->precision, m->h2_stale, m->cfg.past_len, m->cfg.future_len,
+                                     m->cfg.in_channels, m->cfg.out_channels);
+  char tail[64] = "";
+  if (r.kernel == CONV_FIRST && a.src0 == m->x8) snprintf(tail, sizeof tail, " loop_ztiles %d/%d", le.tz_first, a.ntz);
+  if (r.kernel == CONV_FIN && a.out == m->eps_cl && le.zo_end) snprintf(tail, sizeof tail, " loop_planes %d:%d fuse %d", le.zo_first, le.zo_end, le.fuse);
+  snprintf(buf, (size_t)capacity, "conv %s %d %d %d %d %d %d %d %d %d %d %d %d %d %d %d %d %d %d %d %s %d%s", op.label.c_str(), a.ntaps, a.stride, a.par,
            a.C0 + a.C1, a.Co, a.Zo, a.Yo, a.Xo, op.NB, op.MB, a.bz, a.by, a.bx, op.ks,
            (op.small_n ? 1 : 0) | (op.first_k ? 2 : 0) | (op.stat_act ? 4 : 0) | (op.skip_if_fused ? 8 : 0) | (a.CK == 32 ? 16 : 0),
            op.out_act ? op.out_act->C : a.Co,
            a.C0, a.C1, op.wino ? 1 : 0,
-           kConvKernelName[r.kernel], (int)r.form);
+           kConvKernelName[r.kernel], (int)r.form, tail);
+  return 0;
+}
+
+extern "C" int cm_debug_loop_ends(cm_model *m, int32_t mask) {
+  CM_NOT_DIT(m, "cm_debug_loop_ends");
+  if (!m || mask < 0 || mask > 15) return fail("bad argument");
+  m->loop_ends = mask;
   return 0;
 }
 
```

Result: faster. 947.5 denoise-steps/s, aggregate over 1 GPU under weak scaling (every GPU advances its own batch of 64 chains per step), median of 6 (+2.0%).
